# YixunLiang/UniTEX

Hardware: AMD Instinct MI355X
Metric: denoising-steps/sec (higher is better)
Workload: dtype bf16

## Files before the change

### include/unitex_hip.h

```cpp
#ifndef UNITEX_HIP_H
#define UNITEX_HIP_H
#include <stdint.h>
#ifdef __cplusplus
extern "C" {
#endif
#if defined(__GNUC__)
#pragma GCC visibility push(default)
#endif

#define UTX_VERSION 100

typedef struct utx_ctx utx_ctx;
typedef void* utx_stream;

int utx_version(void);
int utx_init(int device, utx_ctx** ctx);
void utx_free(utx_ctx* ctx);
const char* utx_last_error(utx_ctx* ctx);

int utx_set_option(const char* name, int value);
int utx_get_option(const char* name, int* value);
int utx_is_ablation_build(void);


int utx_attn_fwd_bf16(utx_ctx* ctx, const void* q, const void* k, const void* vt, void* o,
                      long q_hs, long q_ss, long k_hs, long k_ss, long vt_hs, long vt_ds, long o_ss,
                      int H, int S, float softmax_scale, utx_stream stream);
int utx_attn_fwd_bf16_kb(utx_ctx* ctx, const void* q, const void* k, const void* vt, void* o,
                         long q_hs, long q_ss, long k_hs, long k_ss, long vt_hs, long vt_ds, long o_ss,
                         int H, int S, float softmax_scale, float key_bias_log2, int key_bias_period, utx_stream stream);
int utx_attn_fwd_bf16_kbq(utx_ctx* ctx, const void* q, const void* k, const void* vt, void* o,
                          long q_hs, long q_ss, long k_hs, long k_ss, long vt_hs, long vt_ds, long o_ss,
                          int H, int S_q, int S_kv, float softmax_scale, float key_bias_log2, int key_bias_period, utx_stream stream);
int utx_attn_fwd_bf16_ws(utx_ctx* ctx, const void* q, const void* k, const void* vt, void* o,
                         long q_hs, long q_ss, long k_hs, long k_ss, long vt_hs, long vt_ds, long o_ss,
                         int H, int S_q, int S_kv, float softmax_scale, float key_bias_log2, int key_bias_period,
                         void* work, size_t work_bytes, utx_stream stream);
size_t utx_attn_workspace_bytes(utx_ctx* ctx, int H, int S_q, int S_kv);

int utx_quant_vt_mx8(utx_ctx* ctx, const void* vt, void* v8, void* vs, int H, int S_pad, utx_stream stream);
int utx_attn_fwd_fp8(utx_ctx* ctx, const void* q8, const void* qs, const void* k8, const void* ks, const void* v8t, const void* vs, void* o, long o_ss,
                     int H, int S_q, int S_kv, int S_pad, float key_bias_log2, int key_bias_period, utx_stream stream);
int utx_attn_fwd_fp8_ws(utx_ctx* ctx, const void* q8, const void* qs, const void* k8, const void* ks, const void* v8t, const void* vs, void* o, long o_ss,
                        int H, int S_q, int S_kv, int S_pad, float key_bias_log2, int key_bias_period, void* work, size_t work_bytes, utx_stream stream);
int utx_attn_plan(int H, int S_q, int S_kv, int n_cus, int out[4]);
int utx_attn_fwd_bf16_blk(utx_ctx* ctx, const void* q, const void* k, const void* vt, void* o,
                          long q_hs, long q_ss, long k_hs, long k_ss, long vt_hs, long vt_ds, long o_ss,
                          int H, int S_q, int S_kv, float softmax_scale, float key_bias_log2, int key_bias_period,
                          void* work, size_t work_bytes, int blk_rows, long q_bs, long k_bs, long vt_bs, utx_stream stream);

typedef struct utx_gemm_desc {
    const void* A; long lda;
    const void* B; long ldb;
    const void* A2; long lda2;
    const void* B2; long ldb2;
    int M, N, K, K2;
    int lora_n_limit;
    int lora_seg_n;
    float alpha;
    const void* bias;
    int gelu_from;
    const void* gate;
    const void* res; long ldres;
    void* C; long ldc;
    int n_split; void* C1; long ldc1;
    int ntn;
    int conv_Hi, conv_Wi, conv_Wo, conv_cin_log2, conv_stride, conv_pad, conv_up;
    const void* zero_page;
    const void* a_scale; long lds_a;
    const void* b_scale; long lds_b;
    int mx8;
    int qk_cols;
    int qk_tok_off;
    float qk_eps, qk_q_scale;
    const void* qk_wq; const void* qk_wk;
    const float* qk_cos; const float* qk_sin;
    void* qk_Qh; void* qk_Kh; long qk_hs;
    void* sk_work; size_t sk_work_bytes;
    void* q_out; long ldq_out;
    void* qs_out; long qs_out_rb;
    int q_out_kt0;
} utx_gemm_desc;
int utx_gemm_bf16(utx_ctx* ctx, const utx_gemm_desc* d, utx_stream stream);
size_t utx_gemm_streamk_workspace_bytes(utx_ctx* ctx);
int utx_gemm_plan(const utx_gemm_desc* d, int n_cus, int out[4]);

int utx_quant_mx8(utx_ctx* ctx, const void* x, long ldx, void* q, long ldq, void* s, long lds, int M, int K, utx_stream stream);
int utx_quant_mx8_packed(utx_ctx* ctx, const void* x, long ldx, void* q, long ldq, void* s, long row_blocks, int M, int K, utx_stream stream);

typedef struct utx_gemv_desc {
    const void* x; long ldx;
    const void* W; long ldw;
    const void* bias;
    void* y; long ldy;
    int M, N, K;
    int silu_in, silu_out;
} utx_gemv_desc;
int utx_gemv_bf16(utx_ctx* ctx, const utx_gemv_desc* d, utx_stream stream);

size_t utx_group_norm_workspace_bytes(void);
int utx_group_norm(utx_ctx* ctx, const void* x, long npix, int C, const void* gamma, const void* beta, float eps, int silu,
                   void* y, void* work, utx_stream stream);
int utx_softmax_rows(utx_ctx* ctx, void* s, long nrow, long ld, int ncol, utx_stream stream);
int utx_conv3x3_thin(utx_ctx* ctx, const void* x, int H, int W, int Cin, const void* wt, const void* bias, int Cout, void* y,
                     utx_stream stream);

typedef struct utx_qkv_post_desc {
    const void* qkv; long ld;
    int q_col, k_col, v_col;
    const void* wq; const void* wk;
    const float* cosb; const float* sinb;
    void* Qh; void* Kh; void* Vt;
    long hs_qk, hs_v, S_pad;
    int n_tok, tok_off, H;
    float eps;
    float q_scale;
    int heads_per_group;
    long gs_qk, gs_v;
    int skip_qk;
    int sub_heads;
    long gs2_qk, gs2_v;
} utx_qkv_post_desc;
int utx_qkv_post(utx_ctx* ctx, const utx_qkv_post_desc* d, utx_stream stream);

int utx_sp_unpack_qkv(utx_ctx* ctx, const void* recv, int P, int Hp, int S_loc, void* q, void* k, void* vt, utx_stream stream);
int utx_sp_unpack_qkv_dedup(utx_ctx* ctx, const void* recv, int P, int Hp, int S_loc, int text_rows, void* q, void* k, void* vt, utx_stream stream);
int utx_sp_unpack_o(utx_ctx* ctx, const void* recv, int P, int Hp, int S_loc, void* out, long ld, utx_stream stream);
int utx_sp_unpack_o_cols(utx_ctx* ctx, const void* recv, int P, int Hp, int S_loc, void* out, long ld, long src_cols, utx_stream stream);

typedef struct utx_ln_mod_desc {
    const void* x; long ldx;
    const void* shift; const void* scale;
    void* y; long ldy;
    int n_tok, D;
    float eps;
    void* q; long ldq;
    void* qs; long qs_row_blocks;
} utx_ln_mod_desc;
int utx_ln_mod(utx_ctx* ctx, const utx_ln_mod_desc* d, utx_stream stream);

typedef struct utx_sched_desc {
    void* x; const void* v; const void* cond;
    long n_noise_elems, n_total_elems;
    float dsigma;
} utx_sched_desc;
int utx_sched_step(utx_ctx* ctx, const utx_sched_desc* d, utx_stream stream);



int utx_transform_points(utx_ctx* ctx, const float* verts, int V, const float* mvp, int n_views,
                         float* clip, float* ndc, utx_stream stream);

long utx_rasterize_workspace_bytes(int F, int H, int W);
int utx_rasterize(utx_ctx* ctx, const float* pos, const int* tri, int F, int H, int W, float* rast,
                  void* work, utx_stream stream);

int utx_interpolate(utx_ctx* ctx, const float* attr, int C, const float* rast, const int* tri, long npix,
                    float* out, utx_stream stream);

int utx_condition_shade(utx_ctx* ctx, const float* rast, const float* nrm, const float* pos, const float* bg3_host,
                        long npix, void* out_normal, void* out_ccm, void* out_alpha, utx_stream stream);

int utx_face_normals(utx_ctx* ctx, const float* verts, const int* faces, int F, float* out, utx_stream stream);

int utx_texture_shade(utx_ctx* ctx, const float* rast, const float* uv, const int* tri, const float* tex, int Ht, int Wt,
                      const float* bg3_host, long npix, void* out, utx_stream stream);

// ... 153 lines not shown
                          int H, int W, void* tmp, void* vis_out, utx_stream stream);

int utx_composite(utx_ctx* ctx, const float* colors, const void* vis, const int* order_host, int n_order, long T,
                  float* atlas, void* winner, utx_stream stream);

int utx_seam_mask(utx_ctx* ctx, const void* winner, const float* rast2d, int H, int W, void* tmp, void* seam, utx_stream stream);
int utx_seam_mask_sized(utx_ctx* ctx, const void* winner, const float* rast2d, int H, int W, int k_boundary, int k_boundary_blur, void* tmp, void* seam,
                        utx_stream stream);

long utx_nn_fill_workspace_bytes(long T);
int utx_nn_fill(utx_ctx* ctx, const float* pos, const void* winner, const float* rast2d, long T, float* atlas,
                int* nn_index, void* work, long work_bytes, utx_stream stream);

int utx_view_visibility(utx_ctx* ctx, const float* attr6, const float* rast, const float* fnormal, const float* dirs, int n, int H, int W,
                        float grad_thr, float cos_thr, int radius, void* tmp, void* vis, float* alpha, utx_stream stream);
int utx_view_visibility_persp(utx_ctx* ctx, const float* attr6, const float* rast, const float* fnormal, const float* eyes, int n, int H, int W,
                              float grad_thr, float cos_thr, int radius, void* tmp, void* vis, float* alpha, utx_stream stream);

typedef struct utx_knn_desc {
    const float* src_pos; const float* src_attr; const float* src_nrm; const unsigned char* src_mask; long N;
    const float* dst_pos; const float* dst_nrm; const unsigned char* dst_mask; long M;
    int k, C, mode;
    float* out_attr; int* out_idx; float* out_d2;
} utx_knn_desc;
long utx_knn_workspace_bytes(long N);
int utx_knn(utx_ctx* ctx, const utx_knn_desc* d, void* work, long work_bytes, utx_stream stream);


long utx_fps_workspace_bytes(long N);
int utx_fps(utx_ctx* ctx, const float* pos, const void* mask, long N, int M, int start, int* out_idx, float* out_d2, void* work, long work_bytes,
            utx_stream stream);
int utx_sample_edges_equal_steps(utx_ctx* ctx, const float* verts, const int* edges, const int* edge_ids, const float* start, const float* length, int E,
                                 float total, long N, float* samples, int* edge_index, float* edge_t, utx_stream stream);
int utx_sample_surface(utx_ctx* ctx, const float* verts, const int* faces, const float* cum, int F, long N, unsigned long long seed, float* samples,
                       int* face_index, float* uvw, utx_stream stream);

int utx_lens_blur_seam(utx_ctx* ctx, const float* src, const void* seam, int H, int W, const float* k49_host, float* dst, utx_stream stream);
int utx_gaussian_blur_seam(utx_ctx* ctx, const float* src, const void* seam, int H, int W, int ksize, const float* w1_host, float* dst, utx_stream stream);

long utx_pull_push_workspace_bytes(int H, int W);
int utx_pull_push(utx_ctx* ctx, const float* kd, const void* mask, int H, int W, float* out, void* work, utx_stream stream);


int utx_backproject_vis(utx_ctx* ctx, const utx_backproject_desc* d, const float* eyes, int sample_mode, utx_bvh* bvh, utx_stream stream);
int utx_composite_winner(utx_ctx* ctx, const void* vis, int n_views, const int* order_host, int n_order, long T, void* winner, utx_stream stream);
int utx_gather_winner(utx_ctx* ctx, const float* rast2d, const int* faces, const float* vndc, const float* images, const void* winner, long T, int V,
                      int n_views, int H, int W, int C, int sample_mode, float* atlas, utx_stream stream);
int utx_nn_fill_c(utx_ctx* ctx, const float* pos, const void* winner, const float* rast2d, long T, int C, float* atlas, int* nn_index,
                  void* work, long work_bytes, utx_stream stream);
int utx_lens_blur_seam_c(utx_ctx* ctx, const float* src, const void* seam, int H, int W, int C, const float* k49_host, float* dst, utx_stream stream);
int utx_gaussian_blur_seam_c(utx_ctx* ctx, const float* src, const void* seam, int H, int W, int C, int ksize, const float* w1_host, float* dst, utx_stream stream);
long utx_pull_push_workspace_bytes_c(int H, int W, int C);
int utx_pull_push_c(utx_ctx* ctx, const float* kd, const void* mask, int H, int W, int C, float* out, void* work, utx_stream stream);

int utx_to_u8(utx_ctx* ctx, const float* src, long n_rows, long row_elems, int flip, void* dst, utx_stream stream);


int utx_chart_flood(utx_ctx* ctx, const int* adj, const int* bucket, int F, int* chart, int* flag, utx_stream stream);

typedef struct utx_plan utx_plan;
int utx_plan_create(utx_ctx* ctx, utx_plan** out);
void utx_plan_free(utx_plan* plan);
int utx_plan_size(const utx_plan* plan);
int utx_plan_add_gemm(utx_plan* plan, const utx_gemm_desc* d);
int utx_plan_add_gemv(utx_plan* plan, const utx_gemv_desc* d);
int utx_plan_add_ln_mod(utx_plan* plan, const utx_ln_mod_desc* d);
int utx_plan_add_qkv_post(utx_plan* plan, const utx_qkv_post_desc* d);
int utx_plan_add_attn(utx_plan* plan, const void* q, const void* k, const void* vt, void* o, long q_hs, long q_ss, long k_hs, long k_ss, long vt_hs,
                      long vt_ds, long o_ss, int H, int S_q, int S_kv, float softmax_scale, float key_bias_log2, int key_bias_period, void* work,
                      size_t work_bytes);
int utx_plan_add_quant_mx8(utx_plan* plan, const void* x, long ldx, void* q, long ldq, void* s, long lds_or_row_blocks, int M, int K, int packed);
int utx_plan_add_add3(utx_plan* plan, const void* a, const void* b, const void* c, void* out, int n);
int utx_plan_add_quant_vt_mx8(utx_plan* plan, const void* vt, void* v8, void* vs, int H, int S_pad);
int utx_plan_add_attn_fp8(utx_plan* plan, const void* q8, const void* qs, const void* k8, const void* ks, const void* v8t, const void* vs, void* o, long o_ss,
                          int H, int S_q, int S_kv, int S_pad, float key_bias_log2, int key_bias_period);
int utx_plan_add_attn_fp8_ws(utx_plan* plan, const void* q8, const void* qs, const void* k8, const void* ks, const void* v8t, const void* vs, void* o, long o_ss,
                             int H, int S_q, int S_kv, int S_pad, float key_bias_log2, int key_bias_period, void* work, size_t work_bytes);
int utx_plan_fork(utx_plan* plan);
int utx_plan_main(utx_plan* plan);
int utx_plan_join(utx_plan* plan);
int utx_plan_run(utx_plan* plan, utx_stream stream, int* failed_entry);
int utx_plan_run_range(utx_plan* plan, int begin, int end, utx_stream stream, int* failed_entry);
int utx_plan_assign_sk(utx_plan* plan, void* sk_work, size_t sk_work_bytes, int n_cus);
int utx_plan_entry(const utx_plan* plan, int i, int* kind, int* side, void* buf, size_t cap);

typedef struct utx_dit_linear {
    const void* w; const void* b;
    const void* lora_A; const void* lora_B;
    float lora_alpha; int lora_rp; int lora_nseg;
    const void* q; const void* s; long lds_s; const void* sp; int sp_row_blocks;
} utx_dit_linear;
typedef struct utx_dit_double_block {
    utx_dit_linear qkv_x, qkv_c, out_x, out_c, ff1_x, ff2_x, ff1_c, ff2_c;
    const void* nq; const void* nk; const void* naq; const void* nak;
    int mod_x, mod_c;
} utx_dit_double_block;
typedef struct utx_dit_single_block {
    utx_dit_linear qkvm, out;
    const void* nq; const void* nk;
    int mod;
} utx_dit_single_block;
typedef struct utx_dit_weights {
    utx_dit_linear x_embedder, context_embedder, proj_out, t_lin1, t_lin2, g_lin1, g_lin2, p_lin1, p_lin2, mod;
    const utx_dit_double_block* dbl; const utx_dit_single_block* sgl;
    int mod_out, n_mod;
} utx_dit_weights;
typedef struct utx_dit_config {
    int num_heads, num_double, num_single, in_channels, joint_dim, pooled_dim, mlp_ratio, guidance_embeds;
    int S_txt, S_img, n_out;
    float key_bias_log2; int key_bias_period;
    int two_streams, n_cus, lora_rank_padded;
    int fp8, fp8_fuse_quant;
} utx_dit_config;
typedef struct utx_dit_workspace {
    void *lat, *enc, *pooled, *tproj, *gproj, *e1, *e_t, *e_g, *e_p, *temb, *mod, *h, *xn, *qkv, *cat, *attn, *out;
    float *cos, *sin;
    void *Qh, *Kh, *Vt, *T, *Tc;
    void* sk_work; size_t sk_work_bytes;
    void* attn_work; size_t attn_work_bytes;
    void *aq, *as_rm, *asp; int asp_row_blocks;
    void *aq2, *asp2; int asp2_row_blocks;
} utx_dit_workspace;
int utx_dit_load(utx_ctx* ctx, const utx_dit_config* cfg, const utx_dit_weights* weights, const utx_dit_workspace* ws, utx_plan** out);
int utx_dit_step(utx_plan* plan, utx_stream stream, int* failed_entry);

int utx_mesh_decimate_qem(const float* verts, int V, const int* faces, int F, int target_faces, double boundary_weight,
                          float* verts_out, int* faces_out, int* V_out, int* F_out);

int utx_abi_sizes(int* out, int n);

#if defined(__GNUC__)
#pragma GCC visibility pop
#endif
#ifdef __cplusplus
}
#endif
#endif
```

### unitex_amd/_lib.py

```python
import ctypes as C
import os

_HERE = os.path.dirname(os.path.abspath(__file__))
LIB_PATH = os.path.join(_HERE, "lib", "libunitex_hip.so")

c_void_p, c_long, c_int, c_float = C.c_void_p, C.c_long, C.c_int, C.c_float


class GemmDesc(C.Structure):
    _fields_ = [("A", c_void_p), ("lda", c_long), ("B", c_void_p), ("ldb", c_long),
                ("A2", c_void_p), ("lda2", c_long), ("B2", c_void_p), ("ldb2", c_long),
                ("M", c_int), ("N", c_int), ("K", c_int), ("K2", c_int),
                ("lora_n_limit", c_int), ("lora_seg_n", c_int), ("alpha", c_float),
                ("bias", c_void_p), ("gelu_from", c_int), ("gate", c_void_p),
                ("res", c_void_p), ("ldres", c_long), ("C", c_void_p), ("ldc", c_long),
                ("n_split", c_int), ("C1", c_void_p), ("ldc1", c_long), ("ntn", c_int),
                ("conv_Hi", c_int), ("conv_Wi", c_int), ("conv_Wo", c_int), ("conv_cin_log2", c_int),
                ("conv_stride", c_int), ("conv_pad", c_int), ("conv_up", c_int), ("zero_page", c_void_p),
                ("a_scale", c_void_p), ("lds_a", c_long), ("b_scale", c_void_p), ("lds_b", c_long), ("mx8", c_int),
                ("qk_cols", c_int), ("qk_tok_off", c_int), ("qk_eps", c_float), ("qk_q_scale", c_float),
                ("qk_wq", c_void_p), ("qk_wk", c_void_p), ("qk_cos", c_void_p), ("qk_sin", c_void_p),
                ("qk_Qh", c_void_p), ("qk_Kh", c_void_p), ("qk_hs", c_long),
                ("sk_work", c_void_p), ("sk_work_bytes", C.c_size_t),
                ("q_out", c_void_p), ("ldq_out", c_long), ("qs_out", c_void_p), ("qs_out_rb", c_long), ("q_out_kt0", c_int)]


class GemvDesc(C.Structure):
    _fields_ = [("x", c_void_p), ("ldx", c_long), ("W", c_void_p), ("ldw", c_long),
                ("bias", c_void_p), ("y", c_void_p), ("ldy", c_long),
                ("M", c_int), ("N", c_int), ("K", c_int), ("silu_in", c_int), ("silu_out", c_int)]


class QkvPostDesc(C.Structure):
    _fields_ = [("qkv", c_void_p), ("ld", c_long), ("q_col", c_int), ("k_col", c_int), ("v_col", c_int),
                ("wq", c_void_p), ("wk", c_void_p), ("cosb", c_void_p), ("sinb", c_void_p),
                ("Qh", c_void_p), ("Kh", c_void_p), ("Vt", c_void_p),
                ("hs_qk", c_long), ("hs_v", c_long), ("S_pad", c_long),
                ("n_tok", c_int), ("tok_off", c_int), ("H", c_int), ("eps", c_float), ("q_scale", c_float),
                ("heads_per_group", c_int), ("gs_qk", c_long), ("gs_v", c_long), ("skip_qk", c_int),
                ("sub_heads", c_int), ("gs2_qk", c_long), ("gs2_v", c_long)]


class LnModDesc(C.Structure):
    _fields_ = [("x", c_void_p), ("ldx", c_long), ("shift", c_void_p), ("scale", c_void_p),
                ("y", c_void_p), ("ldy", c_long), ("n_tok", c_int), ("D", c_int), ("eps", c_float),
                ("q", c_void_p), ("ldq", c_long), ("qs", c_void_p), ("qs_row_blocks", c_long)]


class SchedDesc(C.Structure):
    _fields_ = [("x", c_void_p), ("v", c_void_p), ("cond", c_void_p),
                ("n_noise_elems", c_long), ("n_total_elems", c_long), ("dsigma", c_float)]


class BackprojectDesc(C.Structure):
    _fields_ = [("rast2d", c_void_p), ("verts", c_void_p), ("faces", c_void_p), ("fnormal", c_void_p),
                ("vndc", c_void_p), ("dirs", c_void_p), ("images", c_void_p),
                ("color", c_void_p), ("rayvis", c_void_p), ("alphaok", c_void_p),
                ("T_h", c_int), ("T_w", c_int), ("V", c_int), ("n_views", c_int), ("H", c_int), ("W", c_int),
                ("view_begin", c_int), ("view_count", c_int), ("cos_thresh", c_float), ("two_sqrt3", c_float)]


class KnnDesc(C.Structure):
    _fields_ = [("src_pos", c_void_p), ("src_attr", c_void_p), ("src_nrm", c_void_p), ("src_mask", c_void_p), ("N", c_long),
                ("dst_pos", c_void_p), ("dst_nrm", c_void_p), ("dst_mask", c_void_p), ("M", c_long),
                ("k", c_int), ("C", c_int), ("mode", c_int),
                ("out_attr", c_void_p), ("out_idx", c_void_p), ("out_d2", c_void_p)]


class DitLinear(C.Structure):
    _fields_ = [("w", c_void_p), ("b", c_void_p), ("lora_A", c_void_p), ("lora_B", c_void_p), ("lora_alpha", c_float), ("lora_rp", c_int), ("lora_nseg", c_int),
                ("q", c_void_p), ("s", c_void_p), ("lds_s", c_long), ("sp", c_void_p), ("sp_row_blocks", c_int)]


class DitDoubleBlock(C.Structure):
    _fields_ = [(n, DitLinear) for n in ("qkv_x", "qkv_c", "out_x", "out_c", "ff1_x", "ff2_x", "ff1_c", "ff2_c")] + \
               [("nq", c_void_p), ("nk", c_void_p), ("naq", c_void_p), ("nak", c_void_p), ("mod_x", c_int), ("mod_c", c_int)]


class DitSingleBlock(C.Structure):
    _fields_ = [("qkvm", DitLinear), ("out", DitLinear), ("nq", c_void_p), ("nk", c_void_p), ("mod", c_int)]


class DitWeights(C.Structure):
    _fields_ = [(n, DitLinear) for n in ("x_embedder", "context_embedder", "proj_out", "t_lin1", "t_lin2", "g_lin1", "g_lin2", "p_lin1", "p_lin2", "mod")] + \
               [("dbl", C.POINTER(DitDoubleBlock)), ("sgl", C.POINTER(DitSingleBlock)), ("mod_out", c_int), ("n_mod", c_int)]


class DitConfig(C.Structure):
    _fields_ = [(n, c_int) for n in ("num_heads", "num_double", "num_single", "in_channels", "joint_dim", "pooled_dim", "mlp_ratio", "guidance_embeds",
                                     "S_txt", "S_img", "n_out")] + [("key_bias_log2", c_float), ("key_bias_period", c_int), ("two_streams", c_int), ("n_cus", c_int),
                                                                     ("lora_rank_padded", c_int), ("fp8", c_int), ("fp8_fuse_quant", c_int)]


class DitWorkspace(C.Structure):
    _fields_ = [(n, c_void_p) for n in ("lat", "enc", "pooled", "tproj", "gproj", "e1", "e_t", "e_g", "e_p", "temb", "mod", "h", "xn", "qkv", "cat", "attn", "out",
                                        "cos", "sin", "Qh", "Kh", "Vt", "T", "Tc")] + \
               [("sk_work", c_void_p), ("sk_work_bytes", C.c_size_t), ("attn_work", c_void_p), ("attn_work_bytes", C.c_size_t),
                ("aq", c_void_p), ("as_rm", c_void_p), ("asp", c_void_p), ("asp_row_blocks", c_int), ("aq2", c_void_p), ("asp2", c_void_p), ("asp2_row_blocks", c_int)]


ABI_STRUCTS = [GemmDesc, GemvDesc, QkvPostDesc, LnModDesc, SchedDesc, BackprojectDesc, KnnDesc, DitLinear, DitDoubleBlock, DitSingleBlock, DitWeights, DitConfig,
               DitWorkspace]

SYMBOLS = {
    "utx_version": (c_int, []),
    "utx_init": (c_int, [c_int, C.POINTER(c_void_p)]),
    "utx_free": (None, [c_void_p]),
    "utx_last_error": (C.c_char_p, [c_void_p]),
    "utx_abi_sizes": (c_int, [C.POINTER(c_int), c_int]),
    "utx_plan_create": (c_int, [c_void_p, C.POINTER(c_void_p)]),
    "utx_plan_free": (None, [c_void_p]),
    "utx_plan_size": (c_int, [c_void_p]),
    "utx_plan_add_gemm": (c_int, [c_void_p, C.POINTER(GemmDesc)]),
    "utx_plan_add_gemv": (c_int, [c_void_p, C.POINTER(GemvDesc)]),
    "utx_plan_add_ln_mod": (c_int, [c_void_p, C.POINTER(LnModDesc)]),
    "utx_plan_add_qkv_post": (c_int, [c_void_p, C.POINTER(QkvPostDesc)]),
    "utx_plan_add_attn": (c_int, [c_void_p] * 5 + [c_long] * 7 + [c_int, c_int, c_int, c_float, c_float, c_int, c_void_p, C.c_size_t]),
    "utx_plan_add_quant_mx8": (c_int, [c_void_p, c_void_p, c_long, c_void_p, c_long, c_void_p, c_long, c_int, c_int, c_int]),
    "utx_plan_add_add3": (c_int, [c_void_p, c_void_p, c_void_p, c_void_p, c_void_p, c_int]),
    "utx_plan_add_quant_vt_mx8": (c_int, [c_void_p, c_void_p, c_void_p, c_void_p, c_int, c_int]),
    "utx_plan_add_attn_fp8": (c_int, [c_void_p] * 8 + [c_long, c_int, c_int, c_int, c_int, c_float, c_int]),
    "utx_plan_add_attn_fp8_ws": (c_int, [c_void_p] * 8 + [c_long, c_int, c_int, c_int, c_int, c_float, c_int, c_void_p, C.c_size_t]),
    "utx_plan_fork": (c_int, [c_void_p]),
    "utx_plan_main": (c_int, [c_void_p]),
    "utx_plan_join": (c_int, [c_void_p]),
    "utx_plan_run": (c_int, [c_void_p, c_void_p, C.POINTER(c_int)]),
    "utx_plan_run_range": (c_int, [c_void_p, c_int, c_int, c_void_p, C.POINTER(c_int)]),
    "utx_plan_assign_sk": (c_int, [c_void_p, c_void_p, C.c_size_t, c_int]),
    "utx_plan_entry": (c_int, [c_void_p, c_int, C.POINTER(c_int), C.POINTER(c_int), c_void_p, C.c_size_t]),
    "utx_dit_load": (c_int, [c_void_p, C.POINTER(DitConfig), C.POINTER(DitWeights), C.POINTER(DitWorkspace), C.POINTER(c_void_p)]),
    "utx_dit_step": (c_int, [c_void_p, c_void_p, C.POINTER(c_int)]),
    "utx_mesh_decimate_qem": (c_int, [c_void_p, c_int, c_void_p, c_int, c_int, C.c_double, c_void_p, c_void_p, C.POINTER(c_int), C.POINTER(c_int)]),
    "utx_set_option": (c_int, [C.c_char_p, c_int]),
    "utx_get_option": (c_int, [C.c_char_p, C.POINTER(c_int)]),
    "utx_is_ablation_build": (c_int, []),
    "utx_attn_fwd_bf16": (c_int, [c_void_p] * 5 + [c_long] * 7 + [c_int, c_int, c_float, c_void_p]),
    "utx_attn_fwd_bf16_kb": (c_int, [c_void_p] * 5 + [c_long] * 7 + [c_int, c_int, c_float, c_float, c_int, c_void_p]),
    "utx_attn_fwd_bf16_kbq": (c_int, [c_void_p] * 5 + [c_long] * 7 + [c_int, c_int, c_int, c_float, c_float, c_int, c_void_p]),
    "utx_attn_fwd_bf16_ws": (c_int, [c_void_p] * 5 + [c_long] * 7 + [c_int, c_int, c_int, c_float, c_float, c_int, c_void_p, C.c_size_t, c_void_p]),
    "utx_attn_fwd_bf16_blk": (c_int, [c_void_p] * 5 + [c_long] * 7 + [c_int, c_int, c_int, c_float, c_float, c_int, c_void_p, C.c_size_t, c_int, c_long, c_long, c_long,
                                      c_void_p]),
    "utx_attn_workspace_bytes": (C.c_size_t, [c_void_p, c_int, c_int, c_int]),
    "utx_quant_vt_mx8": (c_int, [c_void_p, c_void_p, c_void_p, c_void_p, c_int, c_int, c_void_p]),
    "utx_attn_fwd_fp8": (c_int, [c_void_p] * 8 + [c_long, c_int, c_int, c_int, c_int, c_float, c_int, c_void_p]),
    "utx_attn_fwd_fp8_ws": (c_int, [c_void_p] * 8 + [c_long, c_int, c_int, c_int, c_int, c_float, c_int, c_void_p, C.c_size_t, c_void_p]),
    "utx_attn_plan": (c_int, [c_int, c_int, c_int, c_int, c_void_p]),
    "utx_gemm_bf16": (c_int, [c_void_p, C.POINTER(GemmDesc), c_void_p]),
    "utx_gemm_streamk_workspace_bytes": (C.c_size_t, [c_void_p]),
    "utx_gemm_plan": (c_int, [C.POINTER(GemmDesc), c_int, C.POINTER(c_int * 4)]),
    "utx_quant_mx8": (c_int, [c_void_p, c_void_p, c_long, c_void_p, c_long, c_void_p, c_long, c_int, c_int, c_void_p]),
    "utx_quant_mx8_packed": (c_int, [c_void_p, c_void_p, c_long, c_void_p, c_long, c_void_p, c_long, c_int, c_int, c_void_p]),
    "utx_gemv_bf16": (c_int, [c_void_p, C.POINTER(GemvDesc), c_void_p]),
    "utx_group_norm_workspace_bytes": (c_long, []),
    "utx_group_norm": (c_int, [c_void_p, c_void_p, c_long, c_int, c_void_p, c_void_p, c_float, c_int, c_void_p, c_void_p, c_void_p]),
    "utx_softmax_rows": (c_int, [c_void_p, c_void_p, c_long, c_long, c_int, c_void_p]),
    "utx_conv3x3_thin": (c_int, [c_void_p, c_void_p, c_int, c_int, c_int, c_void_p, c_void_p, c_int, c_void_p, c_void_p]),
    "utx_qkv_post": (c_int, [c_void_p, C.POINTER(QkvPostDesc), c_void_p]),
    "utx_sp_unpack_qkv": (c_int, [c_void_p, c_void_p, c_int, c_int, c_int, c_void_p, c_void_p, c_void_p, c_void_p]),
    "utx_sp_unpack_qkv_dedup": (c_int, [c_void_p, c_void_p, c_int, c_int, c_int, c_int, c_void_p, c_void_p, c_void_p, c_void_p]),
    "utx_sp_unpack_o": (c_int, [c_void_p, c_void_p, c_int, c_int, c_int, c_void_p, c_long, c_void_p]),
    "utx_sp_unpack_o_cols": (c_int, [c_void_p, c_void_p, c_int, c_int, c_int, c_void_p, c_long, c_long, c_void_p]),
    "utx_ln_mod": (c_int, [c_void_p, C.POINTER(LnModDesc), c_void_p]),
    "utx_sched_step": (c_int, [c_void_p, C.POINTER(SchedDesc), c_void_p]),
    "utx_transform_points": (c_int, [c_void_p, c_void_p, c_int, c_void_p, c_int, c_void_p, c_void_p, c_void_p]),
    "utx_rasterize_workspace_bytes": (c_long, [c_int, c_int, c_int]),
    "utx_rasterize": (c_int, [c_void_p, c_void_p, c_void_p, c_int, c_int, c_int, c_void_p, c_void_p, c_void_p]),
    "utx_interpolate": (c_int, [c_void_p, c_void_p, c_int, c_void_p, c_void_p, c_long, c_void_p, c_void_p]),
    "utx_condition_shade": (c_int, [c_void_p, c_void_p, c_void_p, c_void_p, C.POINTER(c_float), c_long, c_void_p, c_void_p, c_void_p, c_void_p]),
    "utx_face_normals": (c_int, [c_void_p, c_void_p, c_void_p, c_int, c_void_p, c_void_p]),
    "utx_texture_shade": (c_int, [c_void_p, c_void_p, c_void_p, c_void_p, c_void_p, c_int, c_int, C.POINTER(c_float), c_long, c_void_p, c_void_p]),
    "utx_gbuffer_shade": (c_int, [c_void_p, c_int, c_void_p, c_void_p, c_void_p, c_int, c_void_p, c_int, C.POINTER(c_float), c_long, c_void_p, c_void_p, c_void_p]),
    "utx_gbuffer_range": (c_int, [c_void_p, c_int, c_void_p, c_void_p, c_void_p, c_int, c_long, c_void_p, c_void_p, c_void_p]),
    "utx_camera_normals": (c_int, [c_void_p, c_void_p, c_int, c_void_p, c_int, c_void_p, c_void_p]),
    "utx_uv_gbuffer": (c_int, [c_void_p, c_void_p, c_void_p, c_void_p, c_void_p, c_void_p, c_void_p, c_int, c_int, c_int, c_int, C.c_uint, C.POINTER(c_void_p), c_void_p]),
    "utx_screen_gbuffer": (c_int, [c_void_p] * 7 + [c_int] + [c_void_p] * 3 + [c_int] * 5 + [C.POINTER(c_void_p), C.POINTER(c_int), c_int, c_int, c_float, c_void_p, c_void_p,
                                   C.c_uint, C.POINTER(c_void_p), c_void_p]),
    "utx_cubemap_table": (c_int, [c_int, c_float, c_void_p, c_void_p]),
    "utx_latlong_to_cubemap": (c_int, [c_void_p, c_void_p, c_int, c_int, c_int, c_void_p, c_void_p]),
    "utx_cubemap_diffuse": (c_int, [c_void_p, c_void_p, c_int, c_void_p, c_void_p, c_void_p]),
    "utx_cubemap_specular": (c_int, [c_void_p, c_void_p, c_int, c_void_p, c_void_p, c_float, c_float, c_void_p, c_void_p]),
    "utx_dfg_lut": (c_int, [c_void_p, c_int, c_int, c_void_p, c_void_p]),
    "utx_cube_sample": (c_int, [c_void_p, c_void_p, c_int, c_void_p, c_long, c_void_p, c_void_p]),
    "utx_pbr_forward": (c_int, [c_void_p, c_void_p, c_int, c_void_p, c_void_p, c_void_p, c_int, c_void_p, c_void_p, c_int, c_void_p, c_int, c_void_p, c_int, c_long,
                                c_void_p, c_void_p, c_void_p]),
    "utx_pbr_shade": (c_int, [c_void_p, c_void_p, c_void_p, c_void_p, c_void_p, c_void_p, c_void_p, c_int, c_int, c_void_p, c_int, c_int, C.POINTER(c_float),
                              c_void_p, c_int, c_void_p, c_int, c_void_p, c_int, c_float, c_float, C.POINTER(c_float), c_long, c_void_p, c_void_p, c_void_p]),
    "utx_pbr_shading_normal": (c_int, [c_void_p, c_void_p, c_int, c_void_p, c_void_p, c_void_p, c_void_p, c_void_p, c_long, c_void_p, c_void_p]),
    "utx_pbr_shade_nm": (c_int, [c_void_p, c_void_p, c_void_p, c_void_p, c_void_p, c_void_p, c_void_p, c_void_p, c_void_p, c_int, c_int, c_void_p, c_int, c_int,
                                 c_void_p, c_int, c_int, C.POINTER(c_float), c_void_p, c_int, c_void_p, c_int, c_void_p, c_int, c_float, c_float, C.POINTER(c_float),
                                 c_long, c_void_p, c_void_p, c_void_p]),
    "utx_bvh_build": (c_int, [c_void_p, c_void_p, c_int, c_void_p, c_int, C.POINTER(c_void_p), c_void_p]),
    "utx_bvh_workspace_bytes": (C.c_size_t, [c_int]),
    "utx_bvh_build_ws": (c_int, [c_void_p, c_void_p, c_int, c_void_p, c_int, c_void_p, C.c_size_t, C.POINTER(c_void_p), c_void_p]),
    "utx_bvh_free": (None, [c_void_p]),
    "utx_bvh_arrays": (c_int, [c_void_p, C.POINTER(c_void_p), C.POINTER(c_void_p), C.POINTER(c_void_p), C.POINTER(c_void_p)]),
    "utx_bvh_trace": (c_int, [c_void_p, c_void_p, c_void_p, c_void_p, c_long, c_void_p, c_void_p]),
    "utx_visible_faces_rays": (c_int, [c_void_p] * 4 + [c_int, c_void_p, c_int, c_int, c_int, c_void_p, c_void_p, c_void_p]),
    "utx_visible_faces_raster": (c_int, [c_void_p, c_void_p, c_int, c_int, c_int, c_int, c_void_p, c_void_p]),
    "utx_erode_faces": (c_int, [c_void_p, c_void_p, c_void_p, c_int, c_int, c_int, c_int, c_void_p, c_void_p]),
    "utx_visible_vertices": (c_int, [c_void_p, c_void_p, c_void_p, c_int, c_int, c_int, c_void_p, c_void_p]),
    "utx_uv_project": (c_int, [c_void_p, c_void_p, c_void_p, c_int, c_void_p, c_void_p] + [c_int] * 4 + [c_void_p] + [c_int] * 4 + [c_void_p, c_int, c_int, c_float] +
                       [c_void_p] * 5),
    "utx_view_weight_maps": (c_int, [c_void_p, c_void_p, c_void_p, c_int, c_int, c_int, c_int, c_void_p, c_void_p, c_void_p, c_void_p]),
    "utx_vertex_project": (c_int, [c_void_p, c_void_p, c_int, c_void_p, c_int, c_void_p, c_void_p, c_void_p, c_int, c_int, c_void_p, c_int, c_int, c_void_p, c_void_p,
                                   c_int, c_void_p, c_void_p, c_void_p]),
    "utx_vertex_project_blend": (c_int, [c_void_p, c_void_p, c_int, c_void_p, c_int, c_void_p, c_void_p, c_void_p, c_int, c_int, c_void_p, c_int, c_int, c_void_p,
                                         c_void_p, c_int, c_void_p, c_void_p, c_float, c_int, c_float, c_float, c_void_p, c_void_p, c_void_p]),
    "utx_vertex_inpaint_step": (c_int, [c_void_p, c_void_p, c_void_p, c_void_p, c_int, c_void_p, c_void_p, c_void_p, c_void_p, c_void_p, c_void_p]),
    "utx_uv_bake": (c_int, [c_void_p, c_void_p, c_void_p, c_int, c_void_p, c_void_p, c_int, c_int, c_int, c_int, c_void_p, c_void_p, c_void_p, c_int, c_void_p,
                            c_void_p, c_int, c_void_p, c_void_p, c_int, c_float, c_int, c_float, c_float, c_void_p, c_void_p, c_void_p]),
    "utx_uv_dilation_step": (c_int, [c_void_p, c_void_p, c_void_p, c_int, c_int, c_int, c_int, c_void_p, c_void_p, c_void_p, c_void_p]),
    "utx_bvh_trace_count": (c_int, [c_void_p, c_void_p, c_void_p, c_void_p, c_long, c_void_p, c_void_p, c_void_p]),
    "utx_bvh_depth": (c_int, [c_void_p]),
    "utx_backproject": (c_int, [c_void_p, C.POINTER(BackprojectDesc), c_void_p, c_void_p]),
    "utx_backproject_persp": (c_int, [c_void_p, C.POINTER(BackprojectDesc), c_void_p, c_void_p, c_void_p]),
    "utx_backproject_sampled": (c_int, [c_void_p, C.POINTER(BackprojectDesc), c_void_p, c_int, c_void_p, c_void_p]),
    "utx_dilate_visibility": (c_int, [c_void_p, c_void_p, c_void_p, c_void_p, c_int, c_int, c_int, c_void_p, c_void_p, c_void_p]),
    "utx_composite": (c_int, [c_void_p, c_void_p, c_void_p, C.POINTER(c_int), c_int, c_long, c_void_p, c_void_p, c_void_p]),
    "utx_seam_mask": (c_int, [c_void_p, c_void_p, c_void_p, c_int, c_int, c_void_p, c_void_p, c_void_p]),
    "utx_seam_mask_sized": (c_int, [c_void_p, c_void_p, c_void_p, c_int, c_int, c_int, c_int, c_void_p, c_void_p, c_void_p]),
    "utx_view_visibility": (c_int, [c_void_p, c_void_p, c_void_p, c_void_p, c_void_p, c_int, c_int, c_int, c_float, c_float, c_int,
                                    c_void_p, c_void_p, c_void_p, c_void_p]),
    "utx_view_visibility_persp": (c_int, [c_void_p, c_void_p, c_void_p, c_void_p, c_void_p, c_int, c_int, c_int, c_float, c_float, c_int,
                                          c_void_p, c_void_p, c_void_p, c_void_p]),
    "utx_knn_workspace_bytes": (c_long, [c_long]),
    "utx_knn": (c_int, [c_void_p, C.POINTER(KnnDesc), c_void_p, c_long, c_void_p]),
    "utx_fps_workspace_bytes": (c_long, [c_long]),
    "utx_fps": (c_int, [c_void_p, c_void_p, c_void_p, c_long, c_int, c_int, c_void_p, c_void_p, c_void_p, c_long, c_void_p]),
    "utx_sample_edges_equal_steps": (c_int, [c_void_p, c_void_p, c_void_p, c_void_p, c_void_p, c_void_p, c_int, c_float, c_long, c_void_p, c_void_p, c_void_p, c_void_p]),
    "utx_sample_surface": (c_int, [c_void_p, c_void_p, c_void_p, c_void_p, c_int, c_long, C.c_ulonglong, c_void_p, c_void_p, c_void_p, c_void_p]),
    "utx_nn_fill_workspace_bytes": (c_long, [c_long]),
# ... 113 lines not shown
```

### unitex_amd/csrc/build.py

```python
import os
import subprocess
import sys
from concurrent.futures import ThreadPoolExecutor

HERE = os.path.dirname(os.path.abspath(__file__))
LIBDIR = os.path.normpath(os.path.join(HERE, "..", "lib"))
OBJDIR = os.path.join(HERE, "_obj")
HIPCC = os.environ.get("HIPCC", "/opt/rocm/bin/hipcc")
ARCH = "gfx950"

NO_PK = ["-Xclang", "-target-feature", "-Xclang", "-packed-fp32-ops"]

SOURCES = [
    ("attention.hip", []),
    ("attention_glds.hip", ["-fno-slp-vectorize"]),
    ("attention_q64.hip", []),
    ("attention_fp8.hip", NO_PK),
    ("gemm.hip", []),
    ("gemm_w4.hip", []),
    ("dit_elementwise.hip", ["-ffp-contract=off"] + NO_PK),
    ("vae.hip", NO_PK),
    ("capi.cpp", []),
    ("meshproc.cpp", []),
    ("plan.cpp", []),
    ("dit_plan.cpp", []),
]
GEOM = [
    ("raster.hip", ["-ffp-contract=off"]),
    ("gbuffer.hip", ["-ffp-contract=off"] + NO_PK),
    ("pbr.hip", ["-ffp-contract=off"] + NO_PK),
    ("bvh.hip", ["-ffp-contract=off"] + NO_PK),
    ("backproject.hip", ["-ffp-contract=off"] + NO_PK),
    ("vertex_bake.hip", ["-ffp-contract=off"] + NO_PK),
    ("uv_bake.hip", ["-ffp-contract=off"] + NO_PK),
    ("texture_post.hip", ["-ffp-contract=off"] + NO_PK),
    ("knn.hip", ["-ffp-contract=off"]),
    ("sampling.hip", ["-ffp-contract=off"]),
    ("unwrap.hip", []),
]
for s in GEOM:
    if os.path.exists(os.path.join(HERE, s[0])):
        SOURCES.append(s)

COMMON = ["--offload-arch=" + ARCH, "-O3", "-std=c++17", "-fPIC", "-fvisibility=hidden", "-I" + HERE,
          "-I" + os.path.normpath(os.path.join(HERE, "..", "..", "include")), "-x", "hip"]


def _newer(src, obj):
    if not os.path.exists(obj):
        return True
    t = os.path.getmtime(obj)
    deps = [src] + [os.path.join(HERE, h) for h in os.listdir(HERE) if h.endswith(".h") or h.endswith(".inc")]
    deps.append(os.path.normpath(os.path.join(HERE, "..", "..", "include", "unitex_hip.h")))
    return any(os.path.getmtime(d) > t for d in deps)


def _compile(item, objdir=None, defines=()):
    name, extra = item
    objdir = objdir or OBJDIR
    src = os.path.join(HERE, name)
    obj = os.path.join(objdir, name + ".o")
    if _newer(src, obj):
        cmd = [HIPCC] + COMMON + list(defines) + extra + ["-c", src, "-o", obj]
        r = subprocess.run(cmd, capture_output=True, text=True)
        if r.returncode != 0:
            raise RuntimeError("hipcc failed for %s:\n%s" % (name, r.stderr[-4000:]))
    return obj


def build(verbose=True, ablate=False):
    if ablate:
        gen = os.path.normpath(os.path.join(HERE, "..", "..", "tools", "gen_attn_q64.py"))
        r = subprocess.run([sys.executable, gen, "--variants", "--keep-default"], capture_output=True, text=True)
        if r.returncode != 0:
            raise RuntimeError("gen_attn_q64.py failed:\n" + r.stderr[-2000:])
    objdir = OBJDIR + ("_ablate" if ablate else "")
    defines = ["-DUTX_ABLATION"] if ablate else []
    os.makedirs(objdir, exist_ok=True)
    os.makedirs(LIBDIR, exist_ok=True)
    with ThreadPoolExecutor(max_workers=min(8, len(SOURCES))) as ex:
        objs = list(ex.map(lambda it: _compile(it, objdir, defines), SOURCES))
    out = os.path.join(LIBDIR, "libunitex_hip_ablate.so" if ablate else "libunitex_hip.so")
    if (not os.path.exists(out)) or any(os.path.getmtime(o) > os.path.getmtime(out) for o in objs):
        cmd = [HIPCC, "--offload-arch=" + ARCH, "-shared", "-fPIC", "-o", out] + objs
        r = subprocess.run(cmd, capture_output=True, text=True)
        if r.returncode != 0:
            raise RuntimeError("link failed:\n%s" % r.stderr[-4000:])
    if verbose:
        print("built", out)
    return out


if __name__ == "__main__":
    build(ablate="--ablate" in sys.argv)
    sys.exit(0)
```

### unitex_amd/csrc/capi.cpp

```cpp
#include <cstdint>
#include <hip/hip_runtime.h>
#include <stdio.h>
#include <string.h>
#include <string>
#include <stdlib.h>
#include <mutex>
#include <map>
#include <vector>
#include <utility>
#include "kernels.h"
#include "common.h"

UtxOptions g_utx_opt;

struct OptName { const char* name; int UtxOptions::*field; bool ablation; };
static const OptName kOptions[] = {
    {"UTX_ATTN_Q64", &UtxOptions::attn_q64, false},         {"UTX_ATTN_TAILSPLIT", &UtxOptions::attn_tailsplit, false},
    {"UTX_GEMM_GROUP_M", &UtxOptions::gemm_group_m, false}, {"UTX_GEMM_TILE", &UtxOptions::gemm_tile, false},
    {"UTX_GEMM_PERS_GRID", &UtxOptions::gemm_pers_grid, false}, {"UTX_GEMM_STREAMK", &UtxOptions::gemm_streamk, false},
    {"UTX_BVH_STACK_WALK", &UtxOptions::bvh_stack_walk, false}, {"UTX_BVH_PACKET", &UtxOptions::bvh_packet, false},
    {"UTX_ATTN_PEEL", &UtxOptions::attn_peel, false},             {"UTX_ATTN8_PEEL", &UtxOptions::attn8_peel, false},
    {"UTX_NN_GRID", &UtxOptions::nn_grid, false},                 {"UTX_GEMM_FASTK", &UtxOptions::gemm_fastk, false},
    {"UTX_ATTN_VAR", &UtxOptions::attn_var_abl, true},      {"UTX_ATTN_DEBUG", &UtxOptions::attn_debug_abl, true},
    {"UTX_GEMM_DEBUG", &UtxOptions::gemm_debug_abl, true},
// ... 138 lines not shown
                         long q_hs, long q_ss, long k_hs, long k_ss, long vt_hs, long vt_ds, long o_ss,
                         int H, int S, float softmax_scale, float key_bias_log2, int key_bias_period, utx_stream stream) {
    if (!q || !k || !vt || !o) return fail(ctx, -2, "utx_attn_fwd_bf16_kb");
    size_t wsb = 0; void* const ws = ctx_attn_ws(ctx, H, S, S, (hipStream_t)stream, &wsb);
    UTX_CALL(ctx, "utx_attn_fwd_bf16_kb",
             utx_launch_attn_fwd(q, k, vt, o, q_hs, q_ss, k_hs, k_ss, vt_hs, vt_ds, o_ss, H, S, S,
                                 softmax_scale, key_bias_log2, key_bias_period, ws, wsb, (hipStream_t)stream));
}

int utx_attn_fwd_bf16_kbq(utx_ctx* ctx, const void* q, const void* k, const void* vt, void* o,
                          long q_hs, long q_ss, long k_hs, long k_ss, long vt_hs, long vt_ds, long o_ss,
                          int H, int S_q, int S_kv, float softmax_scale, float key_bias_log2, int key_bias_period, utx_stream stream) {
    if (!q || !k || !vt || !o) return fail(ctx, -2, "utx_attn_fwd_bf16_kbq");
    size_t wsb = 0; void* const ws = (S_q > 0) ? ctx_attn_ws(ctx, H, S_q, S_kv, (hipStream_t)stream, &wsb) : nullptr;
    UTX_CALL(ctx, "utx_attn_fwd_bf16_kbq",
             utx_launch_attn_fwd(q, k, vt, o, q_hs, q_ss, k_hs, k_ss, vt_hs, vt_ds, o_ss, H, S_kv, S_q,
                                 softmax_scale, key_bias_log2, key_bias_period, ws, wsb, (hipStream_t)stream));
}

int utx_attn_fwd_bf16_ws(utx_ctx* ctx, const void* q, const void* k, const void* vt, void* o,
                         long q_hs, long q_ss, long k_hs, long k_ss, long vt_hs, long vt_ds, long o_ss,
                         int H, int S_q, int S_kv, float softmax_scale, float key_bias_log2, int key_bias_period,
                         void* work, size_t work_bytes, utx_stream stream) {
    if (!q || !k || !vt || !o) return fail(ctx, -2, "utx_attn_fwd_bf16_ws");
    UTX_CALL(ctx, "utx_attn_fwd_bf16_ws",
             utx_launch_attn_fwd(q, k, vt, o, q_hs, q_ss, k_hs, k_ss, vt_hs, vt_ds, o_ss, H, S_kv, S_q,
                                 softmax_scale, key_bias_log2, key_bias_period, work, work_bytes, (hipStream_t)stream));
}

int utx_attn_fwd_bf16_blk(utx_ctx* ctx, const void* q, const void* k, const void* vt, void* o,
                          long q_hs, long q_ss, long k_hs, long k_ss, long vt_hs, long vt_ds, long o_ss,
                          int H, int S_q, int S_kv, float softmax_scale, float key_bias_log2, int key_bias_period,
                          void* work, size_t work_bytes, int blk_rows, long q_bs, long k_bs, long vt_bs, utx_stream stream) {
    if (!q || !k || !vt || !o || blk_rows <= 0) return fail(ctx, -2, "utx_attn_fwd_bf16_blk");
    UTX_CALL(ctx, "utx_attn_fwd_bf16_blk",
             utx_launch_attn_fwd_blk(q, k, vt, o, q_hs, q_ss, k_hs, k_ss, vt_hs, vt_ds, o_ss, H, S_kv, S_q,
                                     softmax_scale, key_bias_log2, key_bias_period, work, work_bytes, blk_rows, q_bs, k_bs, vt_bs, (hipStream_t)stream));
}

int utx_quant_vt_mx8(utx_ctx* ctx, const void* vt, void* v8, void* vs, int H, int S_pad, utx_stream stream) {
    if (!vt || !v8 || !vs) return fail(ctx, -2, "utx_quant_vt_mx8");
    UTX_CALL(ctx, "utx_quant_vt_mx8", utx_launch_quant_vt_mx8(vt, v8, vs, H, S_pad, (hipStream_t)stream));
}

int utx_attn_fwd_fp8(utx_ctx* ctx, const void* q8, const void* qs, const void* k8, const void* ks, const void* v8t, const void* vs, void* o, long o_ss,
                     int H, int S_q, int S_kv, int S_pad, float key_bias_log2, int key_bias_period, utx_stream stream) {
    if (!q8 || !qs || !k8 || !ks || !v8t || !vs || !o) return fail(ctx, -2, "utx_attn_fwd_fp8");
    Attn8Params p;
    p.q8 = (const uint8_t*)q8; p.k8 = (const uint8_t*)k8; p.v8t = (const uint8_t*)v8t;
    p.qs = (const uint32_t*)qs; p.ks = (const uint32_t*)ks; p.vs = (const uint32_t*)vs;
    p.o = (bf16_t*)o; p.o_ss = o_ss; p.H = H; p.S = S_kv; p.Sq = S_q; p.S_pad = S_pad; p.nqb = 0;
    p.key_bias_log2 = key_bias_log2; p.key_bias_period = key_bias_period;
    p.work = (S_q > 0 && S_q <= S_kv) ? ctx_attn_ws(ctx, H, S_q, S_kv, (hipStream_t)stream, &p.work_bytes) : nullptr;
    if (!p.work) p.work_bytes = 0;
    UTX_CALL(ctx, "utx_attn_fwd_fp8", utx_launch_attn_fwd_fp8(&p, (hipStream_t)stream));
}

int utx_attn_fwd_fp8_ws(utx_ctx* ctx, const void* q8, const void* qs, const void* k8, const void* ks, const void* v8t, const void* vs, void* o, long o_ss,
                        int H, int S_q, int S_kv, int S_pad, float key_bias_log2, int key_bias_period, void* work, size_t work_bytes, utx_stream stream) {
    if (!q8 || !qs || !k8 || !ks || !v8t || !vs || !o) return fail(ctx, -2, "utx_attn_fwd_fp8_ws");
    Attn8Params p;
    p.q8 = (const uint8_t*)q8; p.k8 = (const uint8_t*)k8; p.v8t = (const uint8_t*)v8t;
    p.qs = (const uint32_t*)qs; p.ks = (const uint32_t*)ks; p.vs = (const uint32_t*)vs;
    p.o = (bf16_t*)o; p.o_ss = o_ss; p.H = H; p.S = S_kv; p.Sq = S_q; p.S_pad = S_pad; p.nqb = 0;
    p.key_bias_log2 = key_bias_log2; p.key_bias_period = key_bias_period;
    p.work = work; p.work_bytes = work ? work_bytes : 0;
    UTX_CALL(ctx, "utx_attn_fwd_fp8_ws", utx_launch_attn_fwd_fp8(&p, (hipStream_t)stream));
}

size_t utx_attn_workspace_bytes(utx_ctx* ctx, int H, int S_q, int S_kv) {
    (void)ctx;
    if (H <= 0 || S_kv <= 0 || S_q <= 0) return 0;
    return utx_attn_workspace_bytes_impl(H, S_q == S_kv ? 0 : S_q, S_kv, utx_ncu());
}

int utx_attn_plan(int H, int S_q, int S_kv, int n_cus, int out[4]) {
    if (!out || H <= 0 || S_kv <= 0 || S_q <= 0 || n_cus <= 0) return -2;
    options_from_env_once();
    utx_attn_split_plan_impl(H, S_q == S_kv ? 0 : S_q, S_kv, n_cus, out);
    return 0;
}

size_t utx_gemm_streamk_workspace_bytes(utx_ctx*) { return utx_gemm_streamk_workspace_bytes_impl(); }
int utx_gemm_plan(const utx_gemm_desc* d, int n_cus, int out[4]) {
    if (!d || !out || n_cus <= 0 || d->M <= 0 || d->N <= 0 || d->K <= 0) return -2;
    options_from_env_once();
    return utx_gemm_plan_impl(d, n_cus, d->sk_work != nullptr, out);
}
int utx_gemm_bf16(utx_ctx* ctx, const utx_gemm_desc* d, utx_stream stream) {
    if (!d || !d->A || !d->B || !d->C) return fail(ctx, -2, "utx_gemm_bf16");
    UTX_CALL(ctx, "utx_gemm_bf16", utx_launch_gemm_bf16(d, (hipStream_t)stream));
}

int utx_quant_mx8(utx_ctx* ctx, const void* x, long ldx, void* q, long ldq, void* sc, long lds, int M, int K, utx_stream stream) {
    if (!x || !q || !sc) return fail(ctx, -2, "utx_quant_mx8");
    UTX_CALL(ctx, "utx_quant_mx8", utx_launch_quant_mx8(x, ldx, q, ldq, sc, lds, M, K, (hipStream_t)stream));
}

int utx_quant_mx8_packed(utx_ctx* ctx, const void* x, long ldx, void* q, long ldq, void* sc, long row_blocks, int M, int K, utx_stream stream) {
    if (!x || !q || !sc) return fail(ctx, -2, "utx_quant_mx8_packed");
    UTX_CALL(ctx, "utx_quant_mx8_packed", utx_launch_quant_mx8_packed(x, ldx, q, ldq, sc, row_blocks, M, K, (hipStream_t)stream));
}

int utx_gemv_bf16(utx_ctx* ctx, const utx_gemv_desc* d, utx_stream stream) {
    if (!d || !d->x || !d->W || !d->y) return fail(ctx, -2, "utx_gemv_bf16");
    UTX_CALL(ctx, "utx_gemv_bf16", utx_launch_gemv_bf16(d, (hipStream_t)stream));
}

size_t utx_group_norm_workspace_bytes(void) { return utx_group_norm_workspace_bytes_impl(); }

int utx_group_norm(utx_ctx* ctx, const void* x, long npix, int C, const void* gamma, const void* beta, float eps, int silu,
                   void* y, void* work, utx_stream stream) {
    if (!x || !gamma || !beta || !y || !work) return fail(ctx, -2, "utx_group_norm");
    UTX_CALL(ctx, "utx_group_norm", utx_launch_group_norm(x, npix, C, gamma, beta, eps, silu, y, work, (hipStream_t)stream));
}

int utx_softmax_rows(utx_ctx* ctx, void* s, long nrow, long ld, int ncol, utx_stream stream) {
    if (!s) return fail(ctx, -2, "utx_softmax_rows");
    UTX_CALL(ctx, "utx_softmax_rows", utx_launch_softmax_rows(s, nrow, ld, ncol, (hipStream_t)stream));
}

int utx_conv3x3_thin(utx_ctx* ctx, const void* x, int H, int W, int Cin, const void* wt, const void* bias, int Cout, void* y,
                     utx_stream stream) {
    if (!x || !wt || !bias || !y) return fail(ctx, -2, "utx_conv3x3_thin");
    UTX_CALL(ctx, "utx_conv3x3_thin", utx_launch_conv3x3_thin(x, H, W, Cin, wt, bias, Cout, y, (hipStream_t)stream));
}

int utx_qkv_post(utx_ctx* ctx, const utx_qkv_post_desc* d, utx_stream stream) {
    if (!d || !d->qkv || !d->Qh || !d->Kh || !d->Vt || !d->cosb || !d->sinb || !d->wq || !d->wk)
        return fail(ctx, -2, "utx_qkv_post");
    UTX_CALL(ctx, "utx_qkv_post", utx_launch_qkv_post(d, (hipStream_t)stream));
}

int utx_sp_unpack_qkv(utx_ctx* ctx, const void* recv, int P, int Hp, int S_loc, void* q, void* k, void* vt, utx_stream stream) {
    if (!recv || !q || !k || !vt) return fail(ctx, -2, "utx_sp_unpack_qkv");
    UTX_CALL(ctx, "utx_sp_unpack_qkv", utx_launch_sp_unpack_qkv(recv, P, Hp, S_loc, 0, q, k, vt, (hipStream_t)stream));
}

int utx_sp_unpack_qkv_dedup(utx_ctx* ctx, const void* recv, int P, int Hp, int S_loc, int text_rows, void* q, void* k, void* vt, utx_stream stream) {
    if (!recv || !q || !k || !vt) return fail(ctx, -2, "utx_sp_unpack_qkv_dedup");
    UTX_CALL(ctx, "utx_sp_unpack_qkv_dedup", utx_launch_sp_unpack_qkv(recv, P, Hp, S_loc, text_rows, q, k, vt, (hipStream_t)stream));
}

int utx_sp_unpack_o(utx_ctx* ctx, const void* recv, int P, int Hp, int S_loc, void* out, long ld, utx_stream stream) {
    if (!recv || !out) return fail(ctx, -2, "utx_sp_unpack_o");
    UTX_CALL(ctx, "utx_sp_unpack_o", utx_launch_sp_unpack_o(recv, P, Hp, S_loc, out, ld, 0, (hipStream_t)stream));
}

int utx_sp_unpack_o_cols(utx_ctx* ctx, const void* recv, int P, int Hp, int S_loc, void* out, long ld, long src_cols, utx_stream stream) {
    if (!recv || !out || src_cols <= 0) return fail(ctx, -2, "utx_sp_unpack_o_cols");
    UTX_CALL(ctx, "utx_sp_unpack_o_cols", utx_launch_sp_unpack_o(recv, P, Hp, S_loc, out, ld, src_cols, (hipStream_t)stream));
}

int utx_ln_mod(utx_ctx* ctx, const utx_ln_mod_desc* d, utx_stream stream) {
    if (!d || !d->x || (!d->y && !d->q) || !d->shift || !d->scale) return fail(ctx, -2, "utx_ln_mod");
    UTX_CALL(ctx, "utx_ln_mod", utx_launch_ln_mod(d, (hipStream_t)stream));
}

int utx_sched_step(utx_ctx* ctx, const utx_sched_desc* d, utx_stream stream) {
    if (!d || !d->x || !d->v) return fail(ctx, -2, "utx_sched_step");
    UTX_CALL(ctx, "utx_sched_step", utx_launch_sched_step(d, (hipStream_t)stream));
}


int utx_transform_points(utx_ctx* ctx, const float* verts, int V, const float* mvp, int n_views, float* clip, float* ndc, utx_stream stream) {
    if (!verts || !mvp || !clip) return fail(ctx, -2, "utx_transform_points");
// ... 424 lines not shown
```

### unitex_amd/csrc/common.h

```cpp
#pragma once
#include <hip/hip_runtime.h>
#include <stdint.h>

typedef __attribute__((ext_vector_type(8))) __bf16 bf16x8;
typedef __attribute__((ext_vector_type(4))) __bf16 bf16x4;
typedef __attribute__((ext_vector_type(16))) float f32x16;
typedef __attribute__((ext_vector_type(4))) float f32x4;
typedef __attribute__((ext_vector_type(2))) float f32x2;
#ifndef UTX_BF16_T
#define UTX_BF16_T
typedef uint16_t bf16_t;
#endif

#define UTX_WAVE 64

__device__ __forceinline__ uint16_t f2bf(float f) {
    const __bf16 b = (__bf16)f;
    return __builtin_bit_cast(uint16_t, b);
}
__device__ __forceinline__ float bf2f(uint16_t h) { return __uint_as_float(((uint32_t)h) << 16); }
__device__ __forceinline__ uint32_t pack2bf(float lo, float hi) {
    typedef __attribute__((ext_vector_type(2))) __bf16 bf16x2_t;
    bf16x2_t v;
    v[0] = (__bf16)lo; v[1] = (__bf16)hi;
    return __builtin_bit_cast(uint32_t, v);
}
__device__ __forceinline__ float rbf(float f) { return bf2f(f2bf(f)); }

__device__ __forceinline__ float wave_sum(float v) {
#pragma unroll
    for (int o = 32; o > 0; o >>= 1) v += __shfl_xor(v, o, 64);
    return v;
}
__device__ __forceinline__ float wave_max(float v) {
#pragma unroll
    for (int o = 32; o > 0; o >>= 1) v = fmaxf(v, __shfl_xor(v, o, 64));
    return v;
}

__device__ __forceinline__ int xcd_remap(int bid, int nwg) {
    const int nx = 8;
    int xcd = bid % nx, j = bid / nx;
    int q = nwg / nx, r = nwg % nx;
    int base = (xcd < r) ? xcd * (q + 1) : r * (q + 1) + (xcd - r) * q;
    return base + j;
}

#include <atomic>
static inline int utx_device() { int d = 0; return (hipGetDevice(&d) == hipSuccess && d >= 0 && d < 64) ? d : -1; }
static inline int utx_ncu() {
    static std::atomic<int> tab[64] = {};
    const int d = utx_device();
    int n = d >= 0 ? tab[d].load(std::memory_order_relaxed) : 0;
    if (!n) {
        int cur = 0; hipDeviceProp_t pr;
        n = (hipGetDevice(&cur) == hipSuccess && hipGetDeviceProperties(&pr, cur) == hipSuccess) ? pr.multiProcessorCount : 256;
        if (d >= 0) tab[d].store(n, std::memory_order_relaxed);
    }
    return n;
}
#define UTX_ONCE_PER_DEVICE(flag_) static std::atomic<unsigned long long> flag_{0}; const int flag_##_dev = utx_device(); \
    if (flag_##_dev < 0 || !((flag_.load(std::memory_order_acquire) >> flag_##_dev) & 1ull))
#define UTX_ONCE_DONE(flag_) do { if (flag_##_dev >= 0) flag_.fetch_or(1ull << flag_##_dev, std::memory_order_release); } while (0)
```

### unitex_amd/csrc/dit_plan.cpp

```cpp
#include <hip/hip_runtime.h>
#include <math.h>
#include <string.h>
#include <vector>
#include "kernels.h"

extern "C" {
int utx_plan_assign_sk(utx_plan* p, void* sk_work, size_t sk_work_bytes, int n_cus);
}

namespace {
typedef const char* cptr;
inline cptr off(const void* base, long elems) { return (cptr)base + elems * 2; }

struct Builder {
    utx_plan* plan;
    const utx_dit_config& c;
    const utx_dit_workspace& w;
    int D, H, S, S_pad;
    long Kmax;
    int rc;
    Builder(utx_plan* p, const utx_dit_config& c_, const utx_dit_workspace& w_) : plan(p), c(c_), w(w_), rc(0) {
        H = c.num_heads; D = H * 128; S = c.S_txt + c.S_img; S_pad = (S + 63) / 64 * 64; Kmax = (long)(1 + c.mlp_ratio) * D;
    }
    void chk(int r) { if (r != 0 && rc == 0) rc = r; }

    utx_gemm_desc gemm_desc(const void* A, long lda, int M, int K, const void* B, int N, void* C, long ldc, const void* bias) const {
        utx_gemm_desc d; memset(&d, 0, sizeof(d));
        d.A = A; d.lda = lda; d.B = B; d.ldb = K;
        d.K2 = 0; d.lora_n_limit = 0; d.lora_seg_n = 128;
        d.M = M; d.N = N; d.K = K;
        d.alpha = 1.0f; d.bias = bias; d.gelu_from = N;
        d.C = C; d.ldc = ldc; d.n_split = N;
        return d;
    }
    void add_gemm(utx_gemm_desc d, bool main_stream) { (void)main_stream; chk(utx_plan_add_gemm(plan, &d)); }
    void linear(const utx_dit_linear& L, const void* A, long lda, int M, int K, int N, void* C, long ldc, bool main_stream, const void* T, int lora_limit, int lora_seg,
                int gelu_from = -1, const void* gate = nullptr, const void* res = nullptr, long ldres = 0, int n_split = -1, void* C1 = nullptr, long ldc1 = 0) {
        utx_gemm_desc d = gemm_desc(A, lda, M, K, L.w, N, C, ldc, L.b);
        if (L.lora_A && L.lora_rp > 0) {
            const int nr = L.lora_nseg * L.lora_rp;
            utx_gemm_desc d0 = gemm_desc(A, lda, M, K, L.lora_A, nr, (void*)T, 3L * c.lora_rank_padded, nullptr);
            d0.alpha = L.lora_alpha;
            add_gemm(d0, main_stream);
            d.A2 = T; d.lda2 = 3L * c.lora_rank_padded; d.B2 = L.lora_B; d.ldb2 = L.lora_rp; d.K2 = L.lora_rp;
            d.lora_n_limit = lora_limit > 0 ? lora_limit : N;
            d.lora_seg_n = lora_seg > 0 ? lora_seg : N;
        }
        if (gelu_from >= 0) d.gelu_from = gelu_from;
        d.gate = gate;
        if (gate) { d.res = res; d.ldres = ldres; }
        if (n_split >= 0) d.n_split = n_split;
        if (C1) { d.C1 = C1; d.ldc1 = ldc1; }
        add_gemm(d, main_stream);
    }
    void lnmod(const void* x, void* y, const void* shift, const void* scale, int n_tok, int mxq_row0 = -1) {
        utx_ln_mod_desc d; memset(&d, 0, sizeof(d));
        d.x = x; d.ldx = D; d.shift = shift; d.scale = scale; d.y = y; d.ldy = D; d.n_tok = n_tok; d.D = D; d.eps = 1e-6f;
        if (mxq_row0 >= 0) { d.q = (char*)w.aq + (long)mxq_row0 * Kmax; d.ldq = Kmax; d.qs = w.asp; d.qs_row_blocks = w.asp_row_blocks; }
        chk(utx_plan_add_ln_mod(plan, &d));
    }
    static bool shape_packed(int M, int N, int n_split = -1, int gelu_from = -1) {
        if (N % 256 || (n_split >= 0 && n_split < N && n_split % 256) || (gelu_from >= 0 && gelu_from < N && gelu_from % 256)) return false;
        return (long)((M + 255) / 256) * (N / 256) >= 192;
    }
    bool is_mx(const utx_dit_linear& L) const { return c.fp8 && L.q; }
    bool is_packed(const utx_dit_linear& L, int M, int N, int n_split = -1, int gelu_from = -1) const { return is_mx(L) && L.sp && shape_packed(M, N, n_split, gelu_from); }
    void quant(const void* x, long ldx, void* q, long ldq, void* s, long lds_or_rb, int M, int K, int packed) { chk(utx_plan_add_quant_mx8(plan, x, ldx, q, ldq, s, lds_or_rb, M, K, packed)); }
    struct MxOpt { int quant_cols; int a_col0; bool q_out; MxOpt() : quant_cols(-1), a_col0(0), q_out(false) {} };
    void linear_mx(const utx_dit_linear& L, bool packed, MxOpt o, int row0, const void* A, long lda, int M, int K, int N, void* C, long ldc, int gelu_from = -1,
                   const void* gate = nullptr, const void* res = nullptr, long ldres = 0, int n_split = -1, void* C1 = nullptr, long ldc1 = 0) {
        char* aqv = (char*)w.aq + (long)row0 * Kmax + (packed ? o.a_col0 : 0);
        utx_gemm_desc d = gemm_desc(aqv, Kmax, M, K, L.q, N, C, ldc, L.b);
        if (packed) {
            char* asv = (char*)w.asp + (long)(o.a_col0 / 128) * w.asp_row_blocks * 512;
            const int nq = o.quant_cols < 0 ? K : o.quant_cols;
            if (nq > 0) quant(A, lda, aqv, Kmax, asv, w.asp_row_blocks, M, nq, 1);
            d.a_scale = asv; d.lds_a = w.asp_row_blocks; d.b_scale = L.sp; d.lds_b = L.sp_row_blocks; d.mx8 = 2;
            if (o.q_out) { d.q_out = (char*)w.aq + (long)row0 * Kmax + D; d.ldq_out = Kmax; d.qs_out = w.asp; d.qs_out_rb = w.asp_row_blocks; d.q_out_kt0 = D / 128; }
        } else {
            char* asv = (char*)w.as_rm + (long)row0 * (Kmax / 32);
            quant(A, lda, aqv, Kmax, asv, Kmax / 32, M, K, 0);
            d.a_scale = asv; d.lds_a = Kmax / 32; d.b_scale = L.s; d.lds_b = L.lds_s; d.mx8 = 1;
        }
        if (gelu_from >= 0) d.gelu_from = gelu_from;
        d.gate = gate;
        if (gate) { d.res = res; d.ldres = ldres; }
        if (n_split >= 0) d.n_split = n_split;
        if (C1) { d.C1 = C1; d.ldc1 = ldc1; }
        add_gemm(d, true);
    }
// ... 105 lines not shown
        const bool f_sgl = fuse && p_qkvm && p_out;
        b.lnmod(h, (void*)xn, chunk(o, 0), chunk(o, 1), S, f_sgl ? 0 : -1);
        if (pruned && c.fp8 && B.qkvm.q && B.qkvm.sp && B.out.q && B.out.sp && Builder::shape_packed(n_out, D) && Builder::shape_packed(S, 2 * D)) {
            if (!ws->aq2 || !ws->asp2 || ws->asp2_row_blocks < (n_out + 127) / 128) { b.chk(-2); break; }
            const int r0 = S_txt, r1 = S_txt + n_out;
            const utx_dit_linear& L = B.qkvm;
            cptr Wq = (cptr)L.q, bm = (cptr)L.b;
            const long Kmax = b.Kmax;
            auto sp_rows = [&](const utx_dit_linear& X, int row) { return (const void*)((cptr)X.sp + (long)(row / 128) * 512); };
            auto mx_desc = [&](const void* A, int M, int K, const void* Bq, int N, void* Cc, long ldc, const void* bias, const void* as_, int a_rb, const void* bs_, int b_rb) {
                utx_gemm_desc d = b.gemm_desc(A, Kmax, M, K, Bq, N, Cc, ldc, bias);
                d.a_scale = as_; d.lds_a = a_rb; d.b_scale = bs_; d.lds_b = b_rb; d.mx8 = 2;
                return d;
            };
            b.quant(xn, D, ws->aq, Kmax, ws->asp, ws->asp_row_blocks, S, D, 1);
            b.add_gemm(mx_desc(ws->aq, S, D, Wq + (long)D * D, 2 * D, (void*)off(qkv, D), 3L * D, off(bm, D), ws->asp, ws->asp_row_blocks, sp_rows(L, D), L.sp_row_blocks), true);
            b.quant(off(xn, (long)r0 * D), D, ws->aq2, Kmax, ws->asp2, ws->asp2_row_blocks, n_out, D, 1);
            b.add_gemm(mx_desc(ws->aq2, n_out, D, Wq, D, (void*)off(qkv, (long)r0 * 3 * D), 3L * D, bm, ws->asp2, ws->asp2_row_blocks, sp_rows(L, 0), L.sp_row_blocks), true);
            {
                utx_gemm_desc d = mx_desc(ws->aq2, n_out, D, Wq + 3L * D * D, MR * D, (void*)off(cat, (long)r0 * ldcat + D), ldcat, off(bm, 3L * D), ws->asp2, ws->asp2_row_blocks,
                                          sp_rows(L, 3 * D), L.sp_row_blocks);
                d.gelu_from = 0;
                b.add_gemm(d, true);
            }
            b.qkvpost(qkv, B.nq, B.nk, S, 0);
            b.attn((void*)off(cat, (long)r0 * ldcat), ldcat, r0, r1);
            b.quant(off(cat, (long)r0 * ldcat), ldcat, ws->aq2, Kmax, ws->asp2, ws->asp2_row_blocks, n_out, (int)Kmax, 1);
            {
                utx_gemm_desc d = mx_desc(ws->aq2, n_out, (int)Kmax, B.out.q, D, (void*)off(h, (long)r0 * D), D, B.out.b, ws->asp2, ws->asp2_row_blocks, B.out.sp, B.out.sp_row_blocks);
                d.gate = chunk(o, 2); d.res = off(h, (long)r0 * D); d.ldres = D;
                b.add_gemm(d, true);
            }
            continue;
        }
        if (pruned) {
            const int r0 = S_txt, r1 = S_txt + n_out;
            const utx_dit_linear& L = B.qkvm;
            cptr Wm = (cptr)L.w, bm = (cptr)L.b;
            const bool lora = L.lora_A && L.lora_rp > 0;
            const int R = L.lora_rp;
            const long ldT = 3L * c.lora_rank_padded;
            if (lora) {
                utx_gemm_desc d0 = b.gemm_desc(xn, D, S, D, L.lora_A, 3 * R, (void*)T, ldT, nullptr);
                d0.alpha = L.lora_alpha;
                b.add_gemm(d0, true);
            }
            {
                utx_gemm_desc d = b.gemm_desc(xn, D, S, D, off(Wm, (long)D * D), 2 * D, (void*)off(qkv, D), 3L * D, off(bm, D));
                if (lora) { d.A2 = off(T, R); d.lda2 = ldT; d.B2 = off(L.lora_B, (long)D * R); d.ldb2 = R; d.K2 = R; d.lora_n_limit = 2 * D; d.lora_seg_n = D; }
                b.add_gemm(d, true);
            }
            {
                utx_gemm_desc d = b.gemm_desc(off(xn, (long)r0 * D), D, r1 - r0, D, Wm, D, (void*)off(qkv, (long)r0 * 3 * D), 3L * D, bm);
                if (lora) { d.A2 = off(T, (long)r0 * ldT); d.lda2 = ldT; d.B2 = L.lora_B; d.ldb2 = R; d.K2 = R; d.lora_n_limit = D; d.lora_seg_n = D; }
                b.add_gemm(d, true);
            }
            {
                utx_gemm_desc d = b.gemm_desc(off(xn, (long)r0 * D), D, r1 - r0, D, off(Wm, 3L * D * D), MR * D, (void*)off(cat, (long)r0 * ldcat + D), ldcat, off(bm, 3L * D));
                d.gelu_from = 0;
                b.add_gemm(d, true);
            }
            b.qkvpost(qkv, B.nq, B.nk, S, 0);
            b.attn((void*)off(cat, (long)r0 * ldcat), ldcat, r0, r1);
            {
                utx_gemm_desc d = b.gemm_desc(off(cat, (long)r0 * ldcat), ldcat, r1 - r0, (1 + MR) * D, B.out.w, D, (void*)off(h, (long)r0 * D), D, B.out.b);
                d.gate = chunk(o, 2); d.res = off(h, (long)r0 * D); d.ldres = D;
                b.add_gemm(d, true);
            }
            continue;
        }
        Builder::MxOpt o_qkvm, o_out;
        if (f_sgl) { o_qkvm.quant_cols = 0; o_qkvm.q_out = true; o_out.quant_cols = D; }
        if (x_qkvm) b.linear_mx(B.qkvm, p_qkvm, o_qkvm, 0, xn, D, S, D, (3 + MR) * D, (void*)qkv, 3L * D, 3 * D, nullptr, nullptr, 0, 3 * D, (void*)off(cat, D), ldcat);
        else b.linear(B.qkvm, xn, D, S, D, (3 + MR) * D, (void*)qkv, 3L * D, true, T, 3 * D, D, 3 * D, nullptr, nullptr, 0, 3 * D, (void*)off(cat, D), ldcat);
        b.qkvpost(qkv, B.nq, B.nk, S, 0);
        b.attn((void*)cat, ldcat, 0, S);
        if (x_out) b.linear_mx(B.out, p_out, o_out, 0, cat, ldcat, S, (1 + MR) * D, D, (void*)h, D, -1, chunk(o, 2), h, D);
        else b.linear(B.out, cat, ldcat, S, (1 + MR) * D, D, (void*)h, D, true, T, 0, 0, -1, chunk(o, 2), h, D);
    }
    b.lnmod(h_x, xn_x, chunk(wt->mod_out, 1), chunk(wt->mod_out, 0), n_out);
    b.linear(wt->proj_out, xn_x, D, n_out, D, c.in_channels, ws->out, c.in_channels, true, nullptr, 0, 0);
    if (b.rc) { utx_plan_free(plan); return b.rc; }
    utx_plan_assign_sk(plan, ws->sk_work, ws->sk_work_bytes, ncu);
    *out = plan;
    return 0;
}

extern "C" int utx_dit_step(utx_plan* plan, utx_stream stream, int* failed_entry) { return utx_plan_run(plan, stream, failed_entry); }
```

### unitex_amd/csrc/gemm.hip

```cpp
#include "common.h"
#include "kernels.h"
#include <stdlib.h>

#define GM_BK 64
#define GM_GROUP_M 4

__device__ __forceinline__ float gelu_tanh(float x) {
    const float k0 = 0.7978845608028654f, k1 = 0.044715f;
    const float u = k0 * (x + k1 * x * x * x);
    return x * __builtin_amdgcn_rcpf(1.0f + __expf(-2.0f * u));
}

__device__ __forceinline__ void glds16(const bf16_t* g, char* lds) {
    __builtin_amdgcn_global_load_lds((const __attribute__((address_space(1))) void*)g,
                                     (__attribute__((address_space(3))) void*)lds, 16, 0, 0);
}


#define GM_RES_LOAD1(it_, rowexpr_) rq##it_ = *reinterpret_cast<const uint4*>(pres + (long)(rowexpr_) * p.ldres + gn0);
#define GM_ROW_PASS1(it_, guard_)                                                                                \
    {                                                                                                            \
        const int ml = rrow0 + RPP * (it_);                                                                      \
        const int gm = m0 + 128 * chunk + ml;                                                                    \
        if (guard_) {                                                                                            \
            uint4 yv = *reinterpret_cast<const uint4*>(smem + ml * CROW + rslot * 16);                           \
            if (pgate) {                                                                                         \
                uint32_t yw[4] = {yv.x, yv.y, yv.z, yv.w};                                                       \
                const uint32_t rw[4] = {rq##it_.x, rq##it_.y, rq##it_.z, rq##it_.w};                             \
                _Pragma("unroll") for (int c = 0; c < 4; ++c) {                                                  \
                    const float y0 = bf2f((uint16_t)(yw[c] & 0xffff)), y1 = bf2f((uint16_t)(yw[c] >> 16));       \
                    const float r0 = bf2f((uint16_t)(rw[c] & 0xffff)), r1 = bf2f((uint16_t)(rw[c] >> 16));       \
                    const float o0 = r0 + rbf(gv[2 * c] * y0);                                                   \
                    const float o1 = r1 + rbf(gv[2 * c + 1] * y1);                                               \
                    yw[c] = pack2bf(o0, o1);                                                                     \
                }                                                                                                \
                yv = make_uint4(yw[0], yw[1], yw[2], yw[3]);                                                     \
            }                                                                                                    \
            *reinterpret_cast<uint4*>(cbase + (long)gm * ldc + cn) = yv;                                         \
        }                                                                                                        \
    }

typedef __attribute__((ext_vector_type(8))) int gm_i32x8;
template <int BM, int BN, int NWM, int NWN, bool CONV, bool MX8 = false>
__global__ __launch_bounds__(64 * NWM * NWN, 2) void gemm_bf16_kernel(GemmParams p) {
    constexpr int NW = NWM * NWN, NT = 64 * NW;
    constexpr int WMR = BM / NWM, WNR = BN / NWN;
    constexpr int MI = WMR / 32, NI = WNR / 32;
    constexpr int A_BYTES = BM * GM_BK * 2, B_BYTES = BN * GM_BK * 2, STAGE = A_BYTES + B_BYTES;
    constexpr int CROW = BN * 2 + 16;
    static_assert(BM / 8 / NW == 4 && BN / 8 / NW == 4, "4 A + 4 B global_load_lds per thread per K-step");
    extern __shared__ __attribute__((aligned(16))) char smem[];
    const bf16_t* pA = (const bf16_t*)p.A; const bf16_t* pB = (const bf16_t*)p.B;
    const bf16_t* pA2 = (const bf16_t*)p.A2; const bf16_t* pB2 = (const bf16_t*)p.B2;
    const bf16_t* pbias = (const bf16_t*)p.bias; const bf16_t* pgate = (const bf16_t*)p.gate;
    const bf16_t* pres = (const bf16_t*)p.res;
    bf16_t* pC = (bf16_t*)p.C; bf16_t* pC1 = (bf16_t*)p.C1;
    const int tid = threadIdx.x;
    const int lane = tid & 63;
    const int wave = __builtin_amdgcn_readfirstlane(tid >> 6);
    const int wm = wave / NWN, wn = wave % NWN;
    const int l31 = lane & 31, lh = lane >> 5;

    const int w = xcd_remap(blockIdx.x, gridDim.x);
    const int ntn = p.ntn & 0xffff, group_m = (p.ntn >> 16) & 0xff;
    const int ntm_ = (p.M + BM - 1) / BM;
    const int per_group = group_m * ntn;
    const int grp = w / per_group, rem = w - grp * per_group;
    const int first_tm = grp * group_m;
    const int gsize = (ntm_ - first_tm < group_m) ? ntm_ - first_tm : group_m;
    const int tm = first_tm + rem % gsize, tn = rem / gsize;
    const int m0 = tm * BM, n0 = tn * BN;

    const int nk1 = p.K / GM_BK;
    const bool lora = (p.K2 > 0) && (n0 < p.lora_n_limit);
    const int nk = nk1 + (lora ? p.K2 / GM_BK : 0);
    const long a2_off = lora ? (long)(n0 / p.lora_seg_n) * p.K2 : 0;

    const int srow_in = lane >> 3, sslot = lane & 7;
#define GM_SRC(j_)                                                                                       \
    const int srow##j_ = 8 * (wave + NW * (j_)) + srow_in;                                              \
    const int schunk##j_ = (sslot ^ ((srow##j_ >> 1) & 7)) * 8;                                          \
    const int sgm##j_ = (m0 + srow##j_ > p.M - 1) ? p.M - 1 : m0 + srow##j_;                             \
    const int sgn##j_ = (n0 + srow##j_ > p.N - 1) ? p.N - 1 : n0 + srow##j_;                             \
    const bf16_t* pa##j_ = pA + (long)sgm##j_ * p.lda + schunk##j_;                                      \
    const bf16_t* pb##j_ = pB + (long)sgn##j_ * p.ldb + schunk##j_;
    GM_SRC(0) GM_SRC(1) GM_SRC(2) GM_SRC(3)
    const bf16_t* pzero = (const bf16_t*)p.zero_page;
    const int chlim = CONV ? (p.conv_Hi << p.conv_up) : 0, cwlim = CONV ? (p.conv_Wi << p.conv_up) : 0;
#define GM_CONV_PIX(j_)                                                                                  \
    const int coy##j_ = CONV ? (sgm##j_ / p.conv_Wo) * p.conv_stride - p.conv_pad : 0;                   \
    const int cox##j_ = CONV ? (sgm##j_ % p.conv_Wo) * p.conv_stride - p.conv_pad : 0;
    GM_CONV_PIX(0) GM_CONV_PIX(1) GM_CONV_PIX(2) GM_CONV_PIX(3)
#define GM_CONV_PTR(j_)                                                                                  \
    {                                                                                                    \
// ... 153 lines not shown
                        const uint2 braw = bq[ni][a];
                        bv[0] = bf2f((uint16_t)(braw.x & 0xffff)); bv[1] = bf2f((uint16_t)(braw.x >> 16));
                        bv[2] = bf2f((uint16_t)(braw.y & 0xffff)); bv[3] = bf2f((uint16_t)(braw.y >> 16));
                    }
                    const bool do_gelu = (n0 + nl) >= p.gelu_from;
#pragma unroll
                    for (int mi = 0; mi < MI; ++mi) {
                        float y[4];
#pragma unroll
                        for (int c = 0; c < 4; ++c) {
                            float v = rbf(acc[ni][mi][4 * a + c] * p.alpha + bv[c]);
                            if (do_gelu) v = gelu_tanh(v);
                            y[c] = v;
                        }
                        uint2 o; o.x = pack2bf(y[0], y[1]); o.y = pack2bf(y[2], y[3]);
                        const int ml = wm * WMR + mi * 32 + l31 - 128 * chunk;
                        *reinterpret_cast<uint2*>(smem + ml * CROW + nl * 2) = o;
                    }
                }
            }
        }
        __syncthreads();
        if (gn0 < p.N) {
            GM_ROW_PASS1(0, gm < p.M) GM_ROW_PASS1(1, gm < p.M) GM_ROW_PASS1(2, gm < p.M) GM_ROW_PASS1(3, gm < p.M)
            GM_ROW_PASS1(4, gm < p.M) GM_ROW_PASS1(5, gm < p.M) GM_ROW_PASS1(6, gm < p.M) GM_ROW_PASS1(7, gm < p.M)
        }
    }
}


__device__ __forceinline__ float silu_f(float v) { return v / (1.0f + __expf(-v)); }

__global__ __launch_bounds__(256) void gemv_bf16_kernel(GemvParams p) {
    const int lane = threadIdx.x & 63;
    const int n = blockIdx.x * 4 + (threadIdx.x >> 6);
    if (n >= p.N) return;
    const bf16_t* wrow = (const bf16_t*)p.W + (long)n * p.ldw;
    const bf16_t* pbias = (const bf16_t*)p.bias;
    for (int m = 0; m < p.M; ++m) {
        const bf16_t* xr = (const bf16_t*)p.x + (long)m * p.ldx;
        float s = 0.f;
        for (int k = lane * 8; k < p.K; k += 64 * 8) {
            const uint4 wv = *reinterpret_cast<const uint4*>(wrow + k);
            const uint4 xv = *reinterpret_cast<const uint4*>(xr + k);
            const uint32_t ww[4] = {wv.x, wv.y, wv.z, wv.w};
            const uint32_t xw[4] = {xv.x, xv.y, xv.z, xv.w};
#pragma unroll
            for (int c = 0; c < 4; ++c) {
                float x0 = bf2f((uint16_t)(xw[c] & 0xffff)), x1 = bf2f((uint16_t)(xw[c] >> 16));
                if (p.silu_in) { x0 = rbf(silu_f(x0)); x1 = rbf(silu_f(x1)); }
                s += x0 * bf2f((uint16_t)(ww[c] & 0xffff));
                s += x1 * bf2f((uint16_t)(ww[c] >> 16));
            }
        }
        s = wave_sum(s);
        if (lane == 0) {
            float v = s + (pbias ? bf2f(pbias[n]) : 0.f);
            v = rbf(v);
            if (p.silu_out) v = silu_f(v);
            ((bf16_t*)p.y)[(long)m * p.ldy + n] = f2bf(v);
        }
    }
}

template <int BM, int BN, int NWM, int NWN, bool CONV = false, bool MX8 = false>
static int launch_gemm(GemmParams p, hipStream_t stream, int group_env) {
    constexpr int LDS = 2 * (BM + BN) * GM_BK * 2;
    UTX_ONCE_PER_DEVICE(attr_set) {
        if (hipFuncSetAttribute(reinterpret_cast<const void*>(gemm_bf16_kernel<BM, BN, NWM, NWN, CONV, MX8>),
                                hipFuncAttributeMaxDynamicSharedMemorySize, LDS) != hipSuccess) return -3;
        UTX_ONCE_DONE(attr_set);
    }
    const int ntm = (p.M + BM - 1) / BM;
    const int ntn = (p.N + BN - 1) / BN;
    int group_m = group_env > 0 ? group_env : GM_GROUP_M;
    if (group_m > ntm) group_m = ntm;
    p.ntn = ntn | (group_m << 16);
    hipLaunchKernelGGL((gemm_bf16_kernel<BM, BN, NWM, NWN, CONV, MX8>), dim3(ntm * ntn), dim3(64 * NWM * NWN), LDS, stream, p);
    return hipGetLastError() == hipSuccess ? 0 : -4;
}

static bool gemm_tile_known() {
    const int t = g_utx_opt.gemm_tile;
    return t == 0 || t == 128 || t == 2564;
}

extern "C" int utx_gemm_plan_impl(const GemmParams* pp, int ncu, int sk_has_work, int out[4]) {
    const GemmParams& p = *pp;
    const int tile_env = g_utx_opt.gemm_tile;
    if (!gemm_tile_known()) return -2;
    out[0] = 0; out[1] = ((p.M + 127) / 128) * ((p.N + 127) / 128); out[2] = 0; out[3] = 0;
    if (p.conv_Wo > 0 || p.mx8 == 1) return 0;
    if (p.mx8 != 2) {
        const bool ok256 = (p.N % 256 == 0) && (p.n_split >= p.N || p.n_split % 256 == 0) &&
                           (p.gelu_from >= p.N || p.gelu_from % 256 == 0) &&
                           (p.K2 == 0 || (p.lora_seg_n % 256 == 0 && p.lora_n_limit % 256 == 0));
        const long tiles256 = (long)((p.M + 255) / 256) * ((p.N + 255) / 256);
        if (!ok256 || tile_env == 128 || (tile_env == 0 && tiles256 < 192)) return 0;
        out[1] = (int)tiles256;
    } else {
        out[1] = ((p.M + 255) / 256) * (p.N / 256);
    }
    out[0] = 1;
    int grid = out[1] < ncu ? out[1] : ncu;
    if (g_utx_opt.gemm_pers_grid > 0 && g_utx_opt.gemm_pers_grid < grid) grid = g_utx_opt.gemm_pers_grid;
    utx_gemm_w4_split_plan(&p, out[1], grid, sk_has_work, &out[2], &out[3]);
    return 0;
}

extern "C" int utx_launch_gemm_bf16(const GemmParams* hp, hipStream_t stream) {
    GemmParams p = *hp;
    if (p.M <= 0 || p.N <= 0 || p.K <= 0) return -1;
    if (p.mx8) {
        if (!p.a_scale || !p.b_scale || (p.K % 128) || (p.lda & 15) || (p.ldb & 15) || p.conv_Wo > 0 || p.mx8 > 2) return -2;
        if (p.mx8 == 1 && ((p.lds_a & 3) || (p.lds_b & 3) || p.lds_a < p.K / 32 || p.lds_b < p.K / 32)) return -2;
        p.K /= 2; p.lda /= 2; p.ldb /= 2;
    }
    if ((p.K % GM_BK) || (p.K2 % GM_BK) || (p.N % 8)) return -2;
    if ((p.lda & 7) || (p.ldb & 7) || (p.ldc & 7)) return -2;
    if (p.K2 > 0 && (!p.A2 || !p.B2 || (p.lda2 & 7) || (p.ldb2 & 7) || p.lora_seg_n <= 0 || (p.lora_seg_n % 128))) return -2;
    if (p.gate && (!p.res || (p.ldres & 7))) return -2;
    if (p.n_split < p.N && (!p.C1 || (p.n_split % 128) || (p.ldc1 & 7))) return -2;
    const int group_env = g_utx_opt.gemm_group_m;
    if (!gemm_tile_known()) return -2;
    if (p.qk_cols > 0 && (p.mx8 || p.conv_Wo > 0 || p.gate)) return -2;
    if (p.q_out && p.mx8 != 2) return -2;
    if (p.conv_Wo > 0) {
        if (p.K2 > 0 || !p.zero_page || p.conv_cin_log2 < 6 || p.K != (9 << p.conv_cin_log2) || p.conv_Hi <= 0 || p.conv_Wi <= 0 ||
            p.conv_stride < 1 || p.conv_stride > 2 || p.conv_pad < 0 || p.conv_pad > 1 || (p.conv_up & ~1) || (p.M % p.conv_Wo))
            return -2;
        return launch_gemm<128, 128, 2, 2, true>(p, stream, 0);
    }
    if (p.mx8 == 2) {
        if ((p.N % 256) || (p.n_split < p.N && p.n_split % 256) || (p.gelu_from < p.N && p.gelu_from % 256) || p.K2 > 0 || p.qk_cols > 0) return -2;
        return utx_launch_gemm_w4(p, stream);
    }
    if (p.mx8) return launch_gemm<128, 128, 2, 2, false, true>(p, stream, group_env);
    int plan[4];
    (void)utx_gemm_plan_impl(&p, 256, 1, plan);
    if (p.qk_cols > 0) {
        if ((p.qk_cols % 256) || p.qk_cols > p.N || p.qk_cols > p.n_split || p.qk_cols > p.gelu_from ||
            !p.qk_wq || !p.qk_wk || !p.qk_cos || !p.qk_sin || !p.qk_Qh || !p.qk_Kh || p.qk_hs <= 0 || p.qk_tok_off < 0) return -2;
        if (plan[0] != 1) return -2;
    }
    if (plan[0] == 1) return utx_launch_gemm_w4(p, stream);
    return launch_gemm<128, 128, 2, 2>(p, stream, group_env);
}

extern "C" int utx_launch_gemv_bf16(const GemvParams* hp, hipStream_t stream) {
    GemvParams p = *hp;
    if (!p.x || !p.W || !p.y) return -2;
    if (p.M <= 0 || p.M > 8 || p.N <= 0 || p.K <= 0 || (p.K % 8) || (p.ldw & 7) || (p.ldx & 7)) return -2;
    if ((p.M > 1 && (p.ldx < p.K || p.ldy < p.N)) || (p.N > 1 && p.ldw < p.K)) return -2;
    hipLaunchKernelGGL(gemv_bf16_kernel, dim3((p.N + 3) / 4), dim3(256), 0, stream, p);
    return hipGetLastError() == hipSuccess ? 0 : -4;
}
```

### unitex_amd/csrc/kernels.h

```cpp
#pragma once
#include <hip/hip_runtime.h>
#include <stdint.h>
#include "../../include/unitex_hip.h"
#ifndef UTX_BF16_T
#define UTX_BF16_T
typedef uint16_t bf16_t;
#endif

struct AttnParams {
    const bf16_t* q;
    const bf16_t* k;
    const bf16_t* vt;
    bf16_t* o;
    long q_hs, q_ss, k_hs, k_ss, vt_hs, vt_ds, o_ss;
    int H, S, nqb;
    int Sq;
    int dbg;
    float scale_log2;
    unsigned char* flags;
    int flag_hs;
    int w_base, nsplit, tiles_per_split;
    bf16_t* part_o;
    float* part_lse;
    float key_bias_log2;
    int key_bias_period;
    void* work;
    size_t work_bytes;
    int blk_rows;
    long q_bs, k_bs, vt_bs;
};
struct Attn8Params {
    const uint8_t *q8, *k8;
    const uint8_t* v8t;
    const uint32_t *qs, *ks;
    const uint32_t* vs;
    bf16_t* o;
    long o_ss;
    int H, S, Sq, S_pad, nqb;
    float key_bias_log2;
    int key_bias_period;
    int w_base, nsplit, tiles_per_split;
    bf16_t* part_o;
    float* part_lse;
    void* work;
    size_t work_bytes;
};
struct UtxOptions {
    int attn_q64 = 1;
    int attn_tailsplit = 1;
    int gemm_group_m = 0;
    int gemm_tile = 0;
    int gemm_pers_grid = 0;
    int gemm_streamk = 1;
    int bvh_stack_walk = 0;
    int attn_var_abl = 0, attn_debug_abl = 0, gemm_debug_abl = 0;
    int bvh_packet = 1;
    int attn_peel = 1;
    int attn8_peel = 1;
    int gemm_fastk = 1;
    int nn_grid = 0;
};
extern UtxOptions g_utx_opt;

typedef utx_gemm_desc GemmParams;
typedef utx_knn_desc KnnParams;
typedef utx_gemv_desc GemvParams;
typedef utx_qkv_post_desc QkvPostParams;
typedef utx_ln_mod_desc LnModParams;
typedef utx_sched_desc SchedParams;

extern "C" {
int utx_launch_attn_fwd(const void* q, const void* k, const void* vt, void* o,
                        long q_hs, long q_ss, long k_hs, long k_ss, long vt_hs, long vt_ds,
                        long o_ss, int H, int S, int Sq, float scale, float key_bias_log2, int key_bias_period, void* work, size_t work_bytes, hipStream_t stream);
void utx_attn_split_plan_impl(int H, int Sq, int S, int ncu, int out[4]);
size_t utx_attn_workspace_bytes_impl(int H, int Sq, int S, int ncu);
size_t utx_attn_split_bytes_impl(int H, int Sq, int S, int ncu);
size_t utx_attn_q64_flag_bytes(int H, int Sq, int S);
int utx_attn_q64_takes(const AttnParams* p, int presc);
int utx_launch_attn_merge(const AttnParams* t, int n_items, hipStream_t stream);
int utx_launch_attn_fwd_glds(const AttnParams* p, int presc, hipStream_t stream);
int utx_launch_attn_fwd_fp8(const Attn8Params* p, hipStream_t stream);
int utx_launch_quant_vt_mx8(const void* vt, void* v8, void* vs, int H, int S_pad, hipStream_t stream);
int utx_launch_attn_fwd_blk(const void* q, const void* k, const void* vt, void* o, long q_hs, long q_ss, long k_hs, long k_ss, long vt_hs, long vt_ds,
                            long o_ss, int H, int S, int Sq, float scale, float key_bias_log2, int key_bias_period, void* work, size_t work_bytes,
                            int blk_rows, long q_bs, long k_bs, long vt_bs, hipStream_t stream);
int utx_launch_attn_fwd_q64(const AttnParams* p, int presc, hipStream_t stream);
int utx_launch_gemm_bf16(const GemmParams* p, hipStream_t stream);
size_t utx_gemm_streamk_workspace_bytes_impl(void);
int utx_gemm_plan_impl(const GemmParams* p, int ncu, int sk_has_work, int out[4]);
void utx_gemm_w4_split_plan(const GemmParams* p, int tiles, int grid, int has_work, int* T, int* S);
int utx_launch_gemm_w4(GemmParams p, hipStream_t stream);
int utx_launch_gemv_bf16(const GemvParams* p, hipStream_t stream);
int utx_launch_quant_mx8(const void* x, long ldx, void* q, long ldq, void* s, long lds, int M, int K, hipStream_t stream);
int utx_launch_quant_mx8_packed(const void* x, long ldx, void* q, long ldq, void* s, long row_blocks, int M, int K, hipStream_t stream);
int utx_launch_qkv_post(const QkvPostParams* p, hipStream_t stream);
int utx_launch_sp_unpack_qkv(const void* recv, int P, int Hp, int S_loc, int text_rows, void* q, void* k, void* vt, hipStream_t stream);
int utx_launch_sp_unpack_o(const void* recv, int P, int Hp, int S_loc, void* out, long ld, long src_cols, hipStream_t stream);
size_t utx_group_norm_workspace_bytes_impl(void);
int utx_launch_group_norm(const void* x, long npix, int C, const void* gamma, const void* beta, float eps, int silu, void* y, void* work, hipStream_t stream);
int utx_launch_softmax_rows(void* s, long nrow, long ld, int ncol, hipStream_t stream);
int utx_launch_conv3x3_thin(const void* x, int H, int W, int Cin, const void* wt, const void* bias, int Cout, void* y, hipStream_t stream);
int utx_launch_ln_mod(const LnModParams* p, hipStream_t stream);
int utx_launch_sched_step(const SchedParams* p, hipStream_t stream);
int utx_launch_transform(const float* verts, int V, const float* mvp, int n_views, float* clip, float* ndc, hipStream_t stream);
int utx_launch_rasterize(const float* pos, const int* tri, int F, int H, int W, float* rast, void* work, hipStream_t stream);
int utx_launch_interpolate(const float* attr, int C, const float* rast, const int* tri, long npix, float* out, hipStream_t stream);
int utx_launch_condition_shade(const float* rast, const float* nrm, const float* pos, const float* bg3_host, long npix, void* out_normal, void* out_ccm, void* out_alpha, hipStream_t stream);
int utx_launch_face_normals(const float* verts, const int* faces, int F, float* out, hipStream_t stream);
int utx_launch_view_visibility(const float* attr6, const float* rast, const float* fnormal, const float* dirs, const float* eyes, int n, int H, int W,
                               float grad_thr, float cos_thr, int radius, void* tmp, void* vis, float* alpha, hipStream_t stream);
size_t utx_knn_workspace_bytes_impl(long N);
int utx_launch_knn(const KnnParams* p, void* work, size_t work_bytes, hipStream_t stream);
size_t utx_fps_workspace_bytes_impl(long N);
int utx_launch_fps(const float* pos, const unsigned char* mask, long N, int M, int start, int* out_idx, float* out_d2, void* work, size_t work_bytes, hipStream_t stream);
int utx_launch_sample_edges(const float* verts, const int* edges, const int* edge_ids, const float* start, const float* length, int E, float total, long N,
                            float* samples, int* edge_index, float* edge_t, hipStream_t stream);
int utx_launch_sample_surface(const float* verts, const int* faces, const float* cum, int F, long N, unsigned long long seed, float* samples, int* face_index,
                              float* uvw, hipStream_t stream);
int utx_launch_texture_shade(const float* rast, const float* uv, const int* tri, const float* tex, int Ht, int Wt, const float* bg3_host, long npix, void* out, hipStream_t stream);
int utx_launch_gbuffer_shade(int mode, const float* rast, const int* tri, const float* attr, int stride, const float* scale2, int ndc, int composite, const float* bg3_host, long npix, void* out_u8, float* out_rgba, hipStream_t stream);
int utx_launch_gbuffer_range(int mode, const float* rast, const int* tri, const float* attr, int stride, long npix, float* scale2, int* empty, hipStream_t stream);
int utx_launch_camera_normals(const float* nrm, int V, const float* c2ws, int n_views, float* out, hipStream_t stream);
int utx_launch_uv_gbuffer(const float* rast, const int* tri, const float* v_pos, const float* v_nrm, const float* v_pos_cam, const float* v_nrm_cam, int V, int B, int H2D, int W2D,
                          unsigned want, void* const* outs_host, hipStream_t stream);
int utx_launch_screen_gbuffer(const float* rast, const int* tri, const float* v_pos, const float* v_nrm, const float* v_uv, const float* v_attr, int Ca, const float* clip_w,
                              const float* v_pos_cam, const float* v_nrm_cam, int V, int B, int H, int W, int n_maps, const float* const* maps_host, const int* map_dims_host,
                              int filter, int bg_kind, float bg_scalar, const float* bg_v_attr, const float* bg_map_attr, unsigned want, void* const* outs_host, hipStream_t stream);
int utx_launch_uv_project(const float* rast2d, const int* tri, int F, const unsigned char* face_mask, const float* v_ndc, int V, int B, int H2D, int W2D, const float* map,
                          int Bm, int Hm, int Wm, int C, const float* rast_map, int filter, int bg_kind, float bg_scalar, const float* bg, float* uv, float* uv_alpha,
                          float* map_attr, hipStream_t stream);
int utx_cubemap_table_impl(int N, float costheta_cutoff, float* texels_host, float* tiles_host);
int utx_launch_latlong_to_cubemap(const float* lat, int Hi, int Wi, int N, float* out, hipStream_t stream);
int utx_launch_cubemap_diffuse(const float* cube, int N, const float* texels, float* out, hipStream_t stream);
int utx_launch_cubemap_specular(const float* cube, int N, const float* texels, const float* tiles, float roughness, float costheta_cutoff, float* out, hipStream_t stream);
int utx_launch_dfg_lut(int R, int nsamples, float* out, hipStream_t stream);
int utx_launch_cube_sample(const float* cube, int N, const float* dirs, long n, float* out, hipStream_t stream);
int utx_launch_pbr_forward(const float* eye, int eye_stride, const float* pos, const float* nrm, const float* kd, int kd_stride, const float* ks, const float* light_diffuse, int Nd,
                           const float* light_specular, int Ns, const float* lut, int R, long npix, float* out_diffuse, float* out_specular, hipStream_t stream);
int utx_launch_pbr_shade(const float* rast, const int* tri, const float* vpos, const float* vnrm, const float* vuv, const float* kd, int Hk, int Wk, const float* ks, int Hs, int Ws,
                         const float* eye3_host, const float* light_diffuse, int Nd, const float* light_specular, int Ns, const float* lut, int R, float lambda_diffuse,
                         float lambda_specular, const float* bg3_host, long npix, void* out_u8, float* out_rgba, hipStream_t stream);
int utx_launch_pbr_shading_normal(const float* eye, int eye_stride, const float* pos, const float* pert, const float* snrm, const float* stng, const float* gnrm, long npix,
                                  float* out, hipStream_t stream);
int utx_launch_pbr_shade_nm(const float* rast, const int* tri, const float* vpos, const float* vnrm, const float* vtng, const float* fnrm, const float* vuv, const float* kd, int Hk,
                            int Wk, const float* ks, int Hs, int Ws, const float* nm, int Hn, int Wn, const float* eye3_host, const float* light_diffuse, int Nd,
                            const float* light_specular, int Ns, const float* lut, int R, float lambda_diffuse, float lambda_specular, const float* bg3_host, long npix,
                            void* out_u8, float* out_rgba, hipStream_t stream);
int utx_bvh_build_impl(const float* verts, int V, const int* faces, int F, utx_bvh** out, hipStream_t stream);
size_t utx_bvh_workspace_bytes_impl(int F);
int utx_bvh_build_ws_impl(const float* verts, int V, const int* faces, int F, void* work, size_t work_bytes, utx_bvh** out, hipStream_t stream);
void utx_bvh_free_impl(utx_bvh* b);
int utx_bvh_arrays_impl(utx_bvh* b, int** info, float** aabb, unsigned** codes_sorted, int** idx_sorted);
int utx_bvh_trace_impl(utx_bvh* b, const float* ro, const float* rd, long R, int* tid, unsigned long long* visited, int force_stack, hipStream_t stream);
int utx_bvh_depth_impl(utx_bvh* b);
int utx_visible_faces_rays_impl(utx_bvh* b, const float* verts, const int* faces, int F, const float* c2ws, int B, int perspective, int flags, unsigned char* mask,
                                unsigned long long* visited, hipStream_t stream);
int utx_launch_visible_faces_raster(const float* rast, int B, int H, int W, int F, unsigned char* mask, hipStream_t stream);
int utx_launch_erode_faces(unsigned char* mask, const int* faces, int B, int F, int V, int depth, int* vstamp, hipStream_t stream);
int utx_launch_visible_vertices(const unsigned char* mask, const int* faces, int B, int F, int V, unsigned char* out, hipStream_t stream);
int utx_launch_view_weight_maps(const float* cosn, const float* cam_nrm, int B, int H, int W, int r, void* tmp, float* out, float* arccos_out, hipStream_t stream);
int utx_launch_vertex_project(const float* v_pos, int V, const unsigned char* visible, int B, const float* xform, const float* proj, const float* images, int Hi, int Wi,
                              const float* wmap, int H, int W, const float* v_rgb, const float* weights, int use_alpha, float* acc, float* wacc, float overlay_conf,
                              int blending, float blending_conf, float inpainting_conf, float* blended, unsigned char* inpaint, hipStream_t stream);
int utx_launch_vertex_inpaint_step(const int* rowptr, const int* col, const int* idx, int n, const float* rgb_in, const unsigned char* mask_in, float* rgb_out,
                                   unsigned char* mask_out, int* counter, hipStream_t stream);
int utx_launch_uv_bake(const float* rast2d, const int* faces, int F, const unsigned char* face_mask, const float* v_ndc, int V, int B, int Th, int Tw,
                       const float* images, const float* wmap, const float* rast_view, int R, const float* map_Kd, const float* weights, int use_alpha,
                       float* acc, float* wacc, float overlay_conf, int blending, float blending_conf, float inpainting_conf, float* blended,
                       unsigned char* inpaint, hipStream_t stream);
int utx_launch_uv_dilation_step(const float* col_in, const unsigned char* mask_in, int H, int W, int C, int mode, float* col_out, unsigned char* mask_out,
                                int* counter, hipStream_t stream);
int utx_launch_backproject(const utx_backproject_desc* p, const float* eyes, int sample, const utx_bvh* bvh, hipStream_t stream);
int utx_launch_backproject_vis(const utx_backproject_desc* p, const float* eyes, int sample, const utx_bvh* bvh, hipStream_t stream);
int utx_launch_composite_winner(const void* vis, int n_views, const int* order, int n_order, long T, void* winner, hipStream_t stream);
int utx_launch_gather_winner(const float* rast2d, const int* faces, const float* vndc, const float* images, const void* winner, long T, int V, int n_views, int H, int W, int C, int sample, float* atlas, hipStream_t stream);
// ... 14 lines not shown
```

### unitex_amd/csrc/plan.cpp

```cpp
#include <hip/hip_runtime.h>
#include <string.h>
#include <vector>
#include "kernels.h"

namespace {
enum Kind { K_GEMM, K_GEMV, K_LN_MOD, K_QKV_POST, K_ATTN, K_QUANT, K_ADD3, K_FORK, K_JOIN, K_QUANT_VT, K_ATTN8 };
struct AttnArgs { const void *q, *k, *vt; void* o; long q_hs, q_ss, k_hs, k_ss, vt_hs, vt_ds, o_ss; int H, S_q, S_kv; float scale, kb; int period; void* work; size_t work_bytes; };
struct QuantArgs { const void* x; long ldx; void* q; long ldq; void* s; long lds; int M, K, packed; };
struct Add3Args { const void *a, *b, *c; void* out; int n; };
struct QuantVtArgs { const void* vt; void *v8, *vs; int H, S_pad; };
struct Entry {
    Kind kind; int side;
    union { utx_gemm_desc gemm; utx_gemv_desc gemv; utx_ln_mod_desc ln; utx_qkv_post_desc qkv; AttnArgs attn; QuantArgs quant; Add3Args add3; QuantVtArgs qvt; Attn8Params attn8; };
    Entry() { memset(this, 0, sizeof(*this)); }
};
}

struct utx_plan {
    std::vector<Entry> entries;
    hipStream_t side = nullptr;
    std::vector<hipEvent_t> events;
    int cur_side = 0, open_sections = 0;
    int device = 0;
};
// ... 20 lines not shown

int utx_plan_size(const utx_plan* p) { return p ? (int)p->entries.size() : -2; }

static Entry& push(utx_plan* p, Kind k) { p->entries.emplace_back(); Entry& e = p->entries.back(); e.kind = k; e.side = p->cur_side; return e; }

int utx_plan_add_gemm(utx_plan* p, const utx_gemm_desc* d) { if (!p || !d) return -2; push(p, K_GEMM).gemm = *d; return 0; }
int utx_plan_add_gemv(utx_plan* p, const utx_gemv_desc* d) { if (!p || !d) return -2; push(p, K_GEMV).gemv = *d; return 0; }
int utx_plan_add_ln_mod(utx_plan* p, const utx_ln_mod_desc* d) { if (!p || !d) return -2; push(p, K_LN_MOD).ln = *d; return 0; }
int utx_plan_add_qkv_post(utx_plan* p, const utx_qkv_post_desc* d) { if (!p || !d) return -2; push(p, K_QKV_POST).qkv = *d; return 0; }
int utx_plan_add_attn(utx_plan* p, const void* q, const void* k, const void* vt, void* o, long q_hs, long q_ss, long k_hs, long k_ss, long vt_hs,
                      long vt_ds, long o_ss, int H, int S_q, int S_kv, float softmax_scale, float key_bias_log2, int key_bias_period, void* work,
                      size_t work_bytes) {
    if (!p || !q || !k || !vt || !o) return -2;
    AttnArgs a = {q, k, vt, o, q_hs, q_ss, k_hs, k_ss, vt_hs, vt_ds, o_ss, H, S_q, S_kv, softmax_scale, key_bias_log2, key_bias_period, work, work_bytes};
    push(p, K_ATTN).attn = a;
    return 0;
}
int utx_plan_add_quant_mx8(utx_plan* p, const void* x, long ldx, void* q, long ldq, void* s, long lds_or_row_blocks, int M, int K, int packed) {
    if (!p || !x || !q || !s) return -2;
    QuantArgs a = {x, ldx, q, ldq, s, lds_or_row_blocks, M, K, packed};
    push(p, K_QUANT).quant = a;
    return 0;
}
int utx_plan_add_add3(utx_plan* p, const void* a, const void* b, const void* c, void* out, int n) {
    if (!p || !a || !c || !out || n <= 0) return -2;
    Add3Args g = {a, b, c, out, n};
    push(p, K_ADD3).add3 = g;
    return 0;
}
int utx_plan_add_quant_vt_mx8(utx_plan* p, const void* vt, void* v8, void* vs, int H, int S_pad) {
    if (!p || !vt || !v8 || !vs) return -2;
    QuantVtArgs a = {vt, v8, vs, H, S_pad};
    push(p, K_QUANT_VT).qvt = a;
    return 0;
}
int utx_plan_add_attn_fp8(utx_plan* p, const void* q8, const void* qs, const void* k8, const void* ks, const void* v8t, const void* vs, void* o, long o_ss,
                          int H, int S_q, int S_kv, int S_pad, float key_bias_log2, int key_bias_period) {
    if (!p || !q8 || !qs || !k8 || !ks || !v8t || !vs || !o) return -2;
    Attn8Params a;
    memset(&a, 0, sizeof(a));
    a.q8 = (const uint8_t*)q8; a.k8 = (const uint8_t*)k8; a.v8t = (const uint8_t*)v8t;
    a.qs = (const uint32_t*)qs; a.ks = (const uint32_t*)ks; a.vs = (const uint32_t*)vs;
    a.o = (bf16_t*)o; a.o_ss = o_ss; a.H = H; a.S = S_kv; a.Sq = S_q; a.S_pad = S_pad;
    a.key_bias_log2 = key_bias_log2; a.key_bias_period = key_bias_period;
    push(p, K_ATTN8).attn8 = a;
    return 0;
}
int utx_plan_add_attn_fp8_ws(utx_plan* p, const void* q8, const void* qs, const void* k8, const void* ks, const void* v8t, const void* vs, void* o, long o_ss,
                             int H, int S_q, int S_kv, int S_pad, float key_bias_log2, int key_bias_period, void* work, size_t work_bytes) {
    const int rc = utx_plan_add_attn_fp8(p, q8, qs, k8, ks, v8t, vs, o, o_ss, H, S_q, S_kv, S_pad, key_bias_log2, key_bias_period);
    if (rc) return rc;
    p->entries.back().attn8.work = work;
    p->entries.back().attn8.work_bytes = work ? work_bytes : 0;
    return 0;
}
int utx_plan_fork(utx_plan* p) {
    if (!p || p->cur_side || p->open_sections) return -2;
    if (!p->side && hipStreamCreateWithFlags(&p->side, hipStreamNonBlocking) != hipSuccess) return -5;
    hipEvent_t a, b;
    if (hipEventCreateWithFlags(&a, hipEventDisableTiming) != hipSuccess) return -5;
    if (hipEventCreateWithFlags(&b, hipEventDisableTiming) != hipSuccess) { (void)hipEventDestroy(a); return -5; }
    p->events.push_back(a); p->events.push_back(b);
    push(p, K_FORK);
    p->cur_side = 1; p->open_sections = 1;
    return 0;
}
int utx_plan_main(utx_plan* p) { if (!p || !p->open_sections) return -2; p->cur_side = 0; return 0; }
int utx_plan_join(utx_plan* p) {
    if (!p || !p->open_sections) return -2;
    p->cur_side = 0; p->open_sections = 0;
    push(p, K_JOIN);
    return 0;
}

int utx_plan_assign_sk(utx_plan* p, void* sk_work, size_t sk_work_bytes, int n_cus) {
    if (!p || !sk_work || n_cus <= 0) return 0;
    bool any = false;
    for (const Entry& e : p->entries)
        if (e.kind == K_GEMM && !e.side && (long)((e.gemm.M + 255) / 256) * (e.gemm.N / 256) > n_cus) any = true;
    if (!any) return 0;
    int n = 0;
    for (Entry& e : p->entries)
        if (e.kind == K_GEMM && !e.side) { e.gemm.sk_work = sk_work; e.gemm.sk_work_bytes = sk_work_bytes; ++n; }
    return n;
}

int utx_plan_entry(const utx_plan* p, int i, int* kind, int* side, void* buf, size_t cap) {
    if (!p || i < 0 || i >= (int)p->entries.size() || !kind || !side) return -2;
    const Entry& e = p->entries[i];
    *kind = (int)e.kind; *side = e.side;
    const void* src = nullptr; size_t n = 0;
    switch (e.kind) {
        case K_GEMM: src = &e.gemm; n = sizeof(e.gemm); break;
        case K_GEMV: src = &e.gemv; n = sizeof(e.gemv); break;
        case K_LN_MOD: src = &e.ln; n = sizeof(e.ln); break;
        case K_QKV_POST: src = &e.qkv; n = sizeof(e.qkv); break;
        case K_ATTN: src = &e.attn; n = sizeof(e.attn); break;
        case K_QUANT: src = &e.quant; n = sizeof(e.quant); break;
        case K_ADD3: src = &e.add3; n = sizeof(e.add3); break;
        case K_QUANT_VT: src = &e.qvt; n = sizeof(e.qvt); break;
        case K_ATTN8: src = &e.attn8; n = sizeof(e.attn8); break;
        default: break;
    }
    if (n > cap) return -2;
    if (n && buf) memcpy(buf, src, n);
    return (int)n;
}

int utx_plan_run_range(utx_plan* p, int begin, int end, utx_stream stream_, int* failed_entry) {
    if (!p || p->open_sections || begin < 0 || end > (int)p->entries.size() || begin > end) return -2;
    hipStream_t main_s = (hipStream_t)stream_;
    size_t section = 0;
    int open_at_begin = 0;
    for (int i = 0; i < begin; ++i) {
        if (p->entries[i].kind == K_FORK) ++open_at_begin;
        if (p->entries[i].kind == K_JOIN) { ++section; --open_at_begin; }
    }
    if (open_at_begin != 0) { if (failed_entry) *failed_entry = begin; return -2; }
    bool forked = false;
    int rc = 0, bad = -1;
    for (int i = begin; i < end; ++i) {
        const Entry& e = p->entries[i];
        hipStream_t st = e.side ? p->side : main_s;
        if ((e.side || e.kind == K_JOIN) && !forked) { rc = -2; bad = i; break; }
        switch (e.kind) {
            case K_GEMM: rc = utx_launch_gemm_bf16(&e.gemm, st); break;
            case K_GEMV: rc = utx_launch_gemv_bf16(&e.gemv, st); break;
            case K_LN_MOD: rc = utx_launch_ln_mod(&e.ln, st); break;
            case K_QKV_POST: rc = utx_launch_qkv_post(&e.qkv, st); break;
            case K_ATTN: {
                const AttnArgs& a = e.attn;
                rc = utx_launch_attn_fwd(a.q, a.k, a.vt, a.o, a.q_hs, a.q_ss, a.k_hs, a.k_ss, a.vt_hs, a.vt_ds, a.o_ss, a.H, a.S_kv, a.S_q, a.scale, a.kb,
                                         a.period, a.work, a.work_bytes, st);
                break;
            }
            case K_QUANT: {
                const QuantArgs& a = e.quant;
                rc = a.packed ? utx_launch_quant_mx8_packed(a.x, a.ldx, a.q, a.ldq, a.s, a.lds, a.M, a.K, st)
                              : utx_launch_quant_mx8(a.x, a.ldx, a.q, a.ldq, a.s, a.lds, a.M, a.K, st);
                break;
            }
            case K_ADD3: rc = utx_launch_add3_bf16(e.add3.a, e.add3.b, e.add3.c, e.add3.out, e.add3.n, st); break;
            case K_QUANT_VT: rc = utx_launch_quant_vt_mx8(e.qvt.vt, e.qvt.v8, e.qvt.vs, e.qvt.H, e.qvt.S_pad, st); break;
            case K_ATTN8: rc = utx_launch_attn_fwd_fp8(&e.attn8, st); break;
            case K_FORK:
                if (hipEventRecord(p->events[2 * section], main_s) != hipSuccess || hipStreamWaitEvent(p->side, p->events[2 * section], 0) != hipSuccess) rc = -4;
                else forked = true;
                break;
            case K_JOIN:
                if (hipEventRecord(p->events[2 * section + 1], p->side) != hipSuccess || hipStreamWaitEvent(main_s, p->events[2 * section + 1], 0) != hipSuccess) rc = -4;
                forked = false;
                ++section;
                break;
        }
        if (rc != 0) { bad = i; break; }
    }
    if (rc == 0 && forked) { rc = -2; bad = end; }
    if (forked) {
        if (hipEventRecord(p->events[2 * section + 1], p->side) == hipSuccess) (void)hipStreamWaitEvent(main_s, p->events[2 * section + 1], 0);
    }
    if (rc != 0 && failed_entry) *failed_entry = bad;
    return rc;
}

int utx_plan_run(utx_plan* p, utx_stream stream_, int* failed_entry) {
    if (!p) return -2;
// ... 5 lines not shown
```

### unitex_amd/flux/ops.py

```python
import ctypes as C
import math

import torch

from .. import _lib
from .._lib import GemmDesc, GemvDesc, LnModDesc, QkvPostDesc, SchedDesc, ptr

_CTX = {}


def get_ctx(device=None):
    if device is None:
        device = torch.cuda.current_device()
    if device not in _CTX:
        _CTX[device] = _lib.Context(device)
    return _CTX[device]


def _bf(t):
    assert t.is_cuda and t.dtype == torch.bfloat16, "expected a CUDA bf16 tensor"
    return t


def attention(q, k, vt, S=None, scale=None, out=None, o_ss=None, key_bias_log2=0.0, key_bias_period=0, S_q=None):
# ... 29 lines not shown
    ctx = get_ctx(vt.device.index)
    H, D, S_pad = vt.shape
    assert D == 128 and S_pad % 64 == 0 and vt.is_contiguous()
    v8, vs = out if out is not None else (torch.empty(H, 128, S_pad, dtype=torch.uint8, device=vt.device), torch.empty(H, S_pad // 32, 32, 4, dtype=torch.uint8, device=vt.device))
    ctx.check(ctx.lib.utx_quant_vt_mx8(ctx.handle, ptr(vt), ptr(v8), ptr(vs), H, S_pad, ctx.stream()))
    return v8, vs


def attention_fp8(q8, qs, k8, ks, v8t, vs, S=None, S_q=None, out=None, o_ss=None, key_bias_log2=0.0, key_bias_period=0):
    ctx = get_ctx(q8.device.index)
    H, S_pad, D = q8.shape
    assert D == 128 and v8t.shape == (H, 128, S_pad)
    S = S_pad if S is None else S
    S_q = S if S_q is None else S_q
    if out is None:
        out = torch.empty(S_q, H * 128, dtype=torch.bfloat16, device=q8.device)
    if o_ss is None:
        o_ss = out.stride(0)
    ctx.check(ctx.lib.utx_attn_fwd_fp8(ctx.handle, ptr(q8), ptr(qs), ptr(k8), ptr(ks), ptr(v8t), ptr(vs), ptr(out), o_ss, H, S_q, S, S_pad,
                                       float(key_bias_log2), int(key_bias_period), ctx.stream()))
    return out


def make_gemm_desc(A, B, C_out, bias=None, A2=None, B2=None, lora_n_limit=None, lora_seg_n=None, alpha=1.0,
                   gelu_from=None, gate=None, res=None, n_split=None, C1=None, a_scale=None, b_scale=None, qk_post=None, sk_work=None, q_out=None):
    M, K = A.shape
    N = B.shape[0]
    d = GemmDesc()
    d.A, d.lda, d.B, d.ldb = ptr(A), A.stride(0), ptr(B), B.stride(0)
    if a_scale is not None:
        assert A.dtype == torch.uint8 and B.dtype == torch.uint8 and b_scale is not None
        if hasattr(a_scale, "row_blocks"):
            assert hasattr(b_scale, "row_blocks"), "packed activation scales need packed weight scales"
            d.a_scale, d.lds_a, d.b_scale, d.lds_b, d.mx8 = ptr(a_scale.data), a_scale.row_blocks, ptr(b_scale.data), b_scale.row_blocks, 2
        else:
            d.a_scale, d.lds_a, d.b_scale, d.lds_b, d.mx8 = ptr(a_scale), a_scale.stride(0), ptr(b_scale), b_scale.stride(0), 1
    if A2 is not None:
        d.A2, d.lda2, d.B2, d.ldb2 = ptr(A2), A2.stride(0), ptr(B2), B2.stride(0)
        d.K2 = B2.shape[1]
        d.lora_n_limit = N if lora_n_limit is None else lora_n_limit
        d.lora_seg_n = N if lora_seg_n is None else lora_seg_n
    else:
        d.K2, d.lora_n_limit, d.lora_seg_n = 0, 0, 128
    d.M, d.N, d.K = M, N, K
    if qk_post is not None:
        q = qk_post
        d.qk_cols, d.qk_tok_off, d.qk_eps, d.qk_q_scale = int(q["cols"]), int(q["tok_off"]), float(q["eps"]), float(q["q_scale"])
        d.qk_wq, d.qk_wk, d.qk_cos, d.qk_sin = ptr(q["wq"]), ptr(q["wk"]), ptr(q["cos"]), ptr(q["sin"])
        d.qk_Qh, d.qk_Kh, d.qk_hs = ptr(q["Qh"]), ptr(q["Kh"]), q["Qh"].stride(0)
    d.alpha = alpha
    d.bias = ptr(bias)
    d.gelu_from = N if gelu_from is None else gelu_from
    d.gate = ptr(gate)
    if gate is not None:
        d.res, d.ldres = ptr(res), res.stride(0)
    d.C, d.ldc = ptr(C_out), C_out.stride(0)
    d.n_split = N if n_split is None else n_split
    if C1 is not None:
        d.C1, d.ldc1 = ptr(C1), C1.stride(0)
    if sk_work is not None:
        d.sk_work, d.sk_work_bytes = ptr(sk_work), sk_work.numel() * sk_work.element_size()
    if q_out is not None:
        qv, qs, kt0 = q_out
        d.q_out, d.ldq_out, d.qs_out, d.qs_out_rb, d.q_out_kt0 = ptr(qv), qv.stride(0), ptr(qs), qs.stride(0) // 512, int(kt0)
    return d


_SK_WS = {}


def streamk_workspace(device, stream=None, shared=True):
    dev = torch.device(device)
    ctx = get_ctx(dev.index)
    nbytes = int(ctx.lib.utx_gemm_streamk_workspace_bytes(ctx.handle))
    if not shared:
        return torch.empty(nbytes, dtype=torch.uint8, device=dev)
    st = torch.cuda.current_stream(dev) if stream is None else stream
    key = (dev.index, st.cuda_stream)
    if key not in _SK_WS:
        _SK_WS[key] = torch.empty(nbytes, dtype=torch.uint8, device=dev)
    return _SK_WS[key]


GEMM_KERNELS = ("128x128", "w4")


def gemm_plan(M, N, K=3072, K2=0, n_split=None, gelu_from=None, lora_seg_n=None, lora_n_limit=None, sk=True, n_cus=256):
    lib = _lib.load_library()
    d = GemmDesc()
    d.A = d.B = d.C = 1
    d.M, d.N, d.K, d.K2 = int(M), int(N), int(K), int(K2)
    d.lora_n_limit = (N if lora_n_limit is None else lora_n_limit) if K2 else 0
    d.lora_seg_n = (N if lora_seg_n is None else lora_seg_n) if K2 else 128
    d.n_split = N if n_split is None else n_split
    d.gelu_from = N if gelu_from is None else gelu_from
    d.sk_work = 1 if sk else None
    out = (C.c_int * 4)()
    rc = lib.utx_gemm_plan(C.byref(d), int(n_cus), C.byref(out))
    if rc != 0:
        raise ValueError("utx_gemm_plan -> %d" % rc)
    return {"kernel": GEMM_KERNELS[out[0]], "tiles": out[1], "tail_tiles": out[2], "ranges": out[3]}


def gemm_takes_w4(M, N, n_split=None, gelu_from=None, K2=0, lora_seg_n=None, lora_n_limit=None):
    return gemm_plan(M, N, K2=K2, n_split=n_split, gelu_from=gelu_from, lora_seg_n=lora_seg_n, lora_n_limit=lora_n_limit)["kernel"] == "w4"


def mx8_uses_packed(M, N, n_split=None, gelu_from=None):
    if N % 256 or (n_split is not None and n_split < N and n_split % 256) or (gelu_from is not None and gelu_from < N and gelu_from % 256):
        return False
    return ((M + 255) // 256) * (N // 256) >= 192


def gemm(A, B, bias=None, out=None, **kw):
    ctx = get_ctx(A.device.index)
    M, N = A.shape[0], B.shape[0]
    n_split = kw.get("n_split")
    if out is None:
        out = torch.empty(M, N if n_split is None else n_split, dtype=torch.bfloat16, device=A.device)
    if kw.get("a_scale") is None:
        _bf(A), _bf(B)
    if "sk_work" not in kw and M >= 4096:
        kw = dict(kw, sk_work=streamk_workspace(A.device))
    d = make_gemm_desc(A, B, out, bias=bias, **kw)
    ctx.check(ctx.lib.utx_gemm_bf16(ctx.handle, C.byref(d), ctx.stream()))
    return out


def gemv(x, W, bias=None, silu_in=False, silu_out=False, out=None):
    ctx = get_ctx(x.device.index)
    M, K = x.shape
    N = W.shape[0]
    if out is None:
        out = torch.empty(M, N, dtype=torch.bfloat16, device=x.device)
    d = GemvDesc()
    d.x, d.ldx, d.W, d.ldw, d.bias = ptr(_bf(x)), x.stride(0), ptr(_bf(W)), W.stride(0), ptr(bias)
    d.y, d.ldy, d.M, d.N, d.K = ptr(out), out.stride(0), M, N, K
    d.silu_in, d.silu_out = int(silu_in), int(silu_out)
    ctx.check(ctx.lib.utx_gemv_bf16(ctx.handle, C.byref(d), ctx.stream()))
    return out


def qkv_post(qkv, q_col, k_col, v_col, wq, wk, cos, sin, Qh, Kh, Vt, n_tok, tok_off, H, eps=1e-6, q_scale=1.0,
             heads_per_group=0, group_stride=0, head_stride=None, row_stride_v=None, skip_qk=False, sub_heads=0, sub_stride=0):
    ctx = get_ctx(qkv.device.index)
    d = QkvPostDesc()
    d.qkv, d.ld = ptr(_bf(qkv)), qkv.stride(0)
    d.q_col, d.k_col, d.v_col = q_col, k_col, v_col
    d.wq, d.wk = ptr(_bf(wq)), ptr(_bf(wk))
    assert cos.dtype == torch.float32 and sin.dtype == torch.float32 and cos.is_contiguous()
    d.cosb, d.sinb = ptr(cos), ptr(sin)
    d.Qh, d.Kh, d.Vt = ptr(Qh), ptr(Kh), ptr(Vt)
    if heads_per_group:
        d.hs_qk, d.hs_v, d.S_pad = head_stride, head_stride, row_stride_v
        d.heads_per_group, d.gs_qk, d.gs_v = heads_per_group, group_stride, group_stride
        d.sub_heads, d.gs2_qk, d.gs2_v = sub_heads, sub_stride, sub_stride
    else:
        d.hs_qk, d.hs_v, d.S_pad = Qh.stride(0), Vt.stride(0), Vt.shape[2]
    d.n_tok, d.tok_off, d.H, d.eps, d.q_scale = n_tok, tok_off, H, eps, q_scale
    d.skip_qk = int(bool(skip_qk))
    ctx.check(ctx.lib.utx_qkv_post(ctx.handle, C.byref(d), ctx.stream()))


def ln_mod(x, shift, scale, out=None, eps=1e-6):
    ctx = get_ctx(x.device.index)
    if out is None:
        out = torch.empty_like(x)
# ... 17 lines not shown
```

### unitex_amd/flux/transformer.py

```python
import ctypes as C
import math
import os
from typing import Dict, List, Optional, Tuple

import torch

from .._lib import GemvDesc, LnModDesc, QkvPostDesc, ptr
from . import ops

BF16 = torch.bfloat16

LORA_TARGETS_DOUBLE = ["attn.to_q", "attn.to_k", "attn.to_v", "attn.to_out.0", "attn.add_q_proj",
                       "attn.add_k_proj", "attn.add_v_proj", "attn.to_add_out", "ff.net.0.proj", "ff.net.2",
                       "ff_context.net.0.proj", "ff_context.net.2"]


class FluxShape:

    def __init__(self, num_heads=24, num_double=19, num_single=38, in_channels=64, joint_dim=4096,
                 pooled_dim=768, axes_dim=(16, 56, 56), theta=10000.0, mlp_ratio=4, guidance_embeds=True):
        self.num_heads, self.head_dim = num_heads, 128
        self.num_double, self.num_single = num_double, num_single
        self.in_channels, self.joint_dim, self.pooled_dim = in_channels, joint_dim, pooled_dim
        self.axes_dim, self.theta, self.mlp_ratio = tuple(axes_dim), theta, mlp_ratio
# ... 552 lines not shown
                    a_o = PackedScales(ws["asp2"], n_out, Kmax)
                    plan.append(("quant_mx8", (cat[r0:r1], ws["aq2"], a_o)))
                    plan.append((self.lib.utx_gemm_bf16, ops.make_gemm_desc(ws["aq2"], b["out.q"], h[r0:r1], bias=b["out.b"], gate=g_, res=h[r0:r1],
                                                                            a_scale=a_o, b_scale=b["out.sp"])))
                    continue
                lora = b.get("lora.qkvm")
                kw_kv, kw_q = {}, {}
                if lora is not None:
                    A_cat, B_cat, alpha, _rp = lora
                    R = A_cat.shape[0] // 3
                    Tv = T[:S, : 3 * R]
                    plan.append((self.lib.utx_gemm_bf16, ops.make_gemm_desc(xn, A_cat, Tv, alpha=alpha)))
                    kw_kv = dict(A2=Tv[:, R:], B2=B_cat[D: 3 * D], lora_n_limit=2 * D, lora_seg_n=D)
                    kw_q = dict(A2=Tv[r0:r1, :R], B2=B_cat[:D], lora_n_limit=D, lora_seg_n=D)
                plan.append((self.lib.utx_gemm_bf16, ops.make_gemm_desc(xn, Wm[D: 3 * D], qkv[:, D: 3 * D], bias=bm[D: 3 * D], **kw_kv)))
                plan.append((self.lib.utx_gemm_bf16, ops.make_gemm_desc(xn[r0:r1], Wm[:D], qkv[r0:r1, :D], bias=bm[:D], **kw_q)))
                plan.append((self.lib.utx_gemm_bf16, ops.make_gemm_desc(xn[r0:r1], Wm[3 * D:], cat[r0:r1, D:], bias=bm[3 * D:], gelu_from=0)))
                self._qkvpost(plan, qkv, b["nq"], b["nk"], ws, S, 0)
                self._attn(plan, ws, cat[r0:], S, q_rows=(r0, r1))
                plan.append((self.lib.utx_gemm_bf16, ops.make_gemm_desc(cat[r0:r1], b["out.w"], h[r0:r1], bias=b["out.b"], gate=g_, res=h[r0:r1])))
                continue
            if self.sp is None:
                has_l = b.get("lora.qkvm") is not None
                qkm = qk_fused(S, (3 + sh.mlp_ratio) * D, 0, b["nq"], b["nk"], n_split=3 * D, gelu_from=3 * D, K2=(Rp if has_l else 0),
                               lora_seg_n=D, lora_n_limit=3 * D)
                self._gemm(plan, xn, b["qkvm.w"], qkv, bias=b["qkvm.b"], lora=b.get("lora.qkvm"), lora_n_limit=3 * D,
                           lora_seg_n=D, T=T, gelu_from=3 * D, n_split=3 * D, C1=cat[:, D:], mx8=m_qkvm, qk_post=qkm)
                self._qkvpost(plan, qkv, b["nq"], b["nk"], ws, S, 0, skip_qk=qkm is not None)
            else:
                if sp_mx is not None:
                    Wq, Wsp = sp_mx
                    NW = Wq.shape[0]
                    m_a = (Wq[: 3 * D], Wsp.row_slice(0, 3 * D), ws["aq"], ws["asp"], {"quant_cols": 0 if f_sgl else D})
                    m_b = (Wq[3 * D:], Wsp.row_slice(3 * D, NW), ws["aq"], ws["asp"],
                           dict({"quant_cols": 0}, **({"q_out": (ws["aq"][:S, D:], ws["asp"], D // 128)} if f_sgl else {})))
                else:
                    m_a = m_b = None
                self._gemm(plan, xn, b["qkvm.w"][: 3 * D], qkv, bias=b["qkvm.b"][: 3 * D], lora=b.get("lora.qkvm"),
                           lora_n_limit=3 * D, lora_seg_n=D, T=T, mx8=m_a)
                self._qkvpost(plan, qkv, b["nq"], b["nk"], ws, S, 0)
                plan.append(("sp_start", None))
                self._gemm(plan, xn, b["qkvm.w"][3 * D:], cat[:, D:], bias=b["qkvm.b"][3 * D:], gelu_from=0, mx8=m_b)
            self._attn(plan, ws, cat, S)
            self._gemm(plan, cat, b["out.w"], h, bias=b["out.b"], gate=g_, res=h, mx8=m_out)
        o = self.mod_off[("out",)]
        scale, shift = mod[o: o + D], mod[o + D: o + 2 * D]
        self._lnmod(plan, h_x[:n_out], xn_x[:n_out], shift, scale)
        self._gemm(plan, xn_x[:n_out], W["proj_out.w"], ws["out"][:n_out], bias=W["proj_out.b"])
        self._assign_streamk(plan, ws)
        return {"ws": ws, "plan": plan, "S_txt": S_txt, "S_img": S_img, "n_out": n_out}

    def gemm_census(self, n_cus=None):
        if not self._plans:
            return {}
        if n_cus is None:
            n_cus = torch.cuda.get_device_properties(self.device).multi_processor_count
        out = {}
        arr = (C.c_int * 4)()

        def walk(entries):
            for e in entries:
                if e[0] == "par":
                    walk(e[1][0]); walk(e[1][1])
                elif e[0] is self.lib.utx_gemm_bf16:
                    if self.lib.utx_gemm_plan(C.byref(e[1]), int(n_cus), C.byref(arr)) != 0:
                        continue
                    k = ops.GEMM_KERNELS[arr[0]]
                    out[k] = out.get(k, 0) + 1
                    if arr[2] > 0:
                        out["w4_split_tail"] = out.get("w4_split_tail", 0) + 1
        walk(next(iter(self._plans.values()))["plan"])
        return out

    def _assign_streamk(self, plan, ws):
        ncu = torch.cuda.get_device_properties(self.device).multi_processor_count

        def main_gemms(entries):
            for e in entries:
                if e[0] is self.lib.utx_gemm_bf16:
                    yield e[1]
                elif e[0] == "par":
                    yield from main_gemms(e[1][0])
        descs = list(main_gemms(plan))
        if not any(((d.M + 255) // 256) * (d.N // 256) > ncu for d in descs):
            return
        if "sk" not in ws:
            ws["sk"] = ops.streamk_workspace(self.device, shared=False)
        sk = ws["sk"]
        for d in descs:
            d.sk_work, d.sk_work_bytes = ptr(sk), sk.numel()

    TEXT_KEEP = 64

    def local_text_range(self, S_txt):
        from .ulysses import local_slice
        return (0, S_txt) if self.sp is None else local_slice(S_txt, self.sp[0], self.sp[1])

    def local_image_range(self, S_img):
        from .ulysses import local_slice
        return (0, S_img) if self.sp is None else local_slice(S_img, self.sp[0], self.sp[1])

    def __del__(self):
        try:
            self._drop_plans()
        except Exception:
            pass

    def _drop_plans(self):
        for p in self._plans.values():
            if p.get("cplan") is not None:
                self.lib.utx_plan_free(p["cplan"])
                p["cplan"] = None
        self._plans.clear()
        self._graphs = {}

    def _tproj_device(self, t1000):
        c = self.__dict__.setdefault("_tproj_cache", {})
        t = c.get(t1000)
        if t is None:
            if len(c) > 4096:
                c.clear()
            t = c[t1000] = _timestep_proj(t1000).to(self.device)
        return t

    def set_output_rows(self, n):
        self.out_rows = None if n is None else int(n)

    def set_positions(self, txt_ids, img_ids):
        self._ids = (txt_ids.detach().to("cpu", torch.float32).contiguous(), img_ids.detach().to("cpu", torch.float32).contiguous())
        self.out_rows = None

    def set_conditioning(self, encoder_hidden_states, pooled_projections, guidance: float):
        if self._ids is None:
            raise RuntimeError("set_positions must be called before set_conditioning")
        txt_ids, img_ids = self._ids
        S_txt = encoder_hidden_states.shape[-2]
        assert txt_ids.shape[0] == S_txt, "txt_ids and encoder_hidden_states disagree on the number of text tokens"
        enc = encoder_hidden_states.reshape(S_txt, -1)
        world = 1 if self.sp is None else self.sp[1]
        K = self.TEXT_KEEP
        identical = bool(self.text_dedup and S_txt > K * world and S_txt % (K * world) == 0 and
                         torch.equal(txt_ids, txt_ids[:1].expand_as(txt_ids)) and torch.equal(enc, enc[:1].expand_as(enc)))
        self.sp_kv_dedup = bool(identical and world > 1 and not self.fp8_attention and os.environ.get("UTX_SP_ZERO_COPY", "0") != "1" and
                                os.environ.get("UTX_SP_KV_DEDUP", "1") != "0")
        if identical:
            t0, t1 = 0, K
            self.key_bias_log2 = math.log2(S_txt / float(K * (1 if self.sp_kv_dedup else world)))
            self.text_rows = K
        else:
            t0, t1 = self.local_text_range(S_txt)
            self.key_bias_log2, self.text_rows = 0.0, None
        i0, i1 = self.local_image_range(img_ids.shape[0])
        S_loc = (t1 - t0) + (i1 - i0)
        self.key_bias_period = (S_loc // 64) if (identical and world > 1 and not self.sp_kv_dedup) else 0
        key = (t1 - t0, i1 - i0, self._lora_version, self.key_bias_log2, self.key_bias_period, self.out_rows, self.sp_kv_dedup)
        if key not in self._plans:
            self._drop_plans()
            self._plans[key] = self._build(t1 - t0, i1 - i0)
            if os.environ.get("UTX_C_PLAN", "1") != "0":
                self.compile_plan(self._plans[key])
        p = self._plans[key]
        ws = p["ws"]
        cos, sin = rope_tables(torch.cat([txt_ids[t0:t1], img_ids[i0:i1]], dim=0), self.shape.axes_dim, self.shape.theta)
        ws["cos"].copy_(cos, non_blocking=True)
        ws["sin"].copy_(sin, non_blocking=True)
        ws["enc"].copy_(enc[t0:t1].to(BF16))
        ws["pooled"].copy_(pooled_projections.reshape(1, -1).to(BF16))
        g1000 = _bf16_scalar(_bf16_scalar(guidance) * 1000.0)
        ws["gproj"].copy_(_timestep_proj(g1000))

    def _launch(self, fn, d, st, timed=True):
        gev = self.gemm_events
        if gev is not None and timed and fn is self.lib.utx_gemm_bf16 and d.M >= 4096:
# ... 181 lines not shown
        if not ok:
            lib.utx_plan_free(h)
            return None
        if segments is not None:
            segments.append((seg_begin, int(lib.utx_plan_size(h)), None))
        old = p.get("cplan")
        if old is not None:
            lib.utx_plan_free(old)
        p["cplan"] = h
        p["segments"] = segments
        return h

    def _run_segments(self, p):
        st, ws = self.ctx.stream(), p["ws"]
        bad = C.c_int(-1)
        for b0, b1, host_op in p["segments"]:
            if b1 > b0:
                rc = self.lib.utx_plan_run_range(p["cplan"], b0, b1, st, C.byref(bad))
                if rc:
                    raise RuntimeError("utx_plan_run_range [%d, %d): entry %d failed with code %d" % (b0, b1, bad.value, rc))
            if host_op is not None:
                self._sp_entry(host_op[0], host_op[1], ws, st)

    def build_c_dit_plan(self, p=None):
        from .._lib import DitConfig, DitDoubleBlock, DitLinear, DitSingleBlock, DitWeights, DitWorkspace
        if self.sp is not None or self.fuse_qk or self.fp8_attention:
            return None
        p = next(iter(self._plans.values())) if p is None else p
        ws, sh, W = p["ws"], self.shape, self.W

        def lin(w, b_, lora=None, blk=None, nm=None):
            L = DitLinear()
            L.w, L.b = ptr(w), ptr(b_)
            if lora is not None:
                A_cat, B_cat, alpha, Rp = lora
                L.lora_A, L.lora_B, L.lora_alpha, L.lora_rp, L.lora_nseg = ptr(A_cat), ptr(B_cat), float(alpha), int(Rp), A_cat.shape[0] // Rp
            if self.fp8_weights and blk is not None and (nm + ".q") in blk:
                L.q, L.s, L.lds_s = ptr(blk[nm + ".q"]), ptr(blk[nm + ".s"]), blk[nm + ".s"].stride(0)
                sp = blk.get(nm + ".sp")
                if sp is not None:
                    L.sp, L.sp_row_blocks = ptr(sp.data), sp.row_blocks
            return L
        wt = DitWeights()
        wt.x_embedder = lin(self._w("x_embedder.w"), self._w("x_embedder.b"))
        wt.context_embedder = lin(W["context_embedder.w"], W["context_embedder.b"])
        wt.proj_out = lin(W["proj_out.w"], W["proj_out.b"])
        k = "time_text_embed.%s.%s"
        for dst, nm in (("t", "timestep_embedder"), ("g", "guidance_embedder"), ("p", "text_embedder")):
            if nm == "guidance_embedder" and not sh.guidance_embeds:
                continue
            for j in (1, 2):
                setattr(wt, "%s_lin%d" % (dst, j), lin(W[k % (nm, "linear_%d" % j) + ".w"], W[k % (nm, "linear_%d" % j) + ".b"]))
        wt.mod = lin(W["mod.w"], W["mod.b"])
        dbl = (DitDoubleBlock * max(1, len(self.double)))()
        for i, b in enumerate(self.double):
            for nm in ("qkv_x", "qkv_c", "out_x", "out_c", "ff1_x", "ff2_x", "ff1_c", "ff2_c"):
                setattr(dbl[i], nm, lin(b[nm + ".w"], b[nm + ".b"], b.get("lora." + nm), b, nm))
            dbl[i].nq, dbl[i].nk, dbl[i].naq, dbl[i].nak = ptr(b["nq"]), ptr(b["nk"]), ptr(b["naq"]), ptr(b["nak"])
            dbl[i].mod_x, dbl[i].mod_c = self.mod_off[("d", i, "x")], self.mod_off[("d", i, "c")]
        sgl = (DitSingleBlock * max(1, len(self.single)))()
        for i, b in enumerate(self.single):
            sgl[i].qkvm = lin(b["qkvm.w"], b["qkvm.b"], b.get("lora.qkvm"), b, "qkvm")
            sgl[i].out = lin(b["out.w"], b["out.b"], None, b, "out")
            sgl[i].nq, sgl[i].nk, sgl[i].mod = ptr(b["nq"]), ptr(b["nk"]), self.mod_off[("s", i)]
        wt.dbl, wt.sgl = dbl, sgl
        wt.mod_out, wt.n_mod = self.mod_off[("out",)], self.n_mod
        cfg = DitConfig()
        cfg.num_heads, cfg.num_double, cfg.num_single = sh.num_heads, sh.num_double, sh.num_single
        cfg.in_channels, cfg.joint_dim, cfg.pooled_dim, cfg.mlp_ratio, cfg.guidance_embeds = sh.in_channels, sh.joint_dim, sh.pooled_dim, sh.mlp_ratio, int(sh.guidance_embeds)
        cfg.S_txt, cfg.S_img, cfg.n_out = p["S_txt"], p["S_img"], p["n_out"]
        cfg.key_bias_log2, cfg.key_bias_period = float(self.key_bias_log2), int(self.key_bias_period)
        cfg.two_streams = int(bool(self.overlap_text))
        cfg.n_cus = torch.cuda.get_device_properties(self.device).multi_processor_count
        cfg.lora_rank_padded = int(self.lora_rank) if self._lora_active else 0
        cfg.fp8 = int(bool(self.fp8_weights))
        cfg.fp8_fuse_quant = int(bool(self.fp8_weights) and os.environ.get("UTX_FP8_FUSE_QUANT", "1") != "0")
        w = DitWorkspace()
        for nm in ("lat", "enc", "pooled", "tproj", "gproj", "e1", "e_t", "e_g", "e_p", "temb", "mod", "h", "xn", "qkv", "cat", "attn", "out", "cos", "sin", "Qh", "Kh",
                   "Vt", "T", "Tc"):
            setattr(w, nm, ptr(ws.get(nm)))
        sk, aw = ws.get("sk"), ws.get("attn_ws")
        w.sk_work, w.sk_work_bytes = ptr(sk), 0 if sk is None else sk.numel()
        w.attn_work, w.attn_work_bytes = ptr(aw), 0 if aw is None else aw.numel()
        if self.fp8_weights:
            w.aq, w.as_rm, w.asp, w.asp_row_blocks = ptr(ws["aq"]), ptr(ws["as"]), ptr(ws["asp"]), ws["asp"].stride(0) // 512
            if "aq2" in ws:
                w.aq2, w.asp2, w.asp2_row_blocks = ptr(ws["aq2"]), ptr(ws["asp2"]), ws["asp2"].stride(0) // 512
        h = C.c_void_p()
        self.ctx.check(self.lib.utx_dit_load(self.ctx.handle, C.byref(cfg), C.byref(wt), C.byref(w), C.byref(h)))
        return h

    def forward(self, hidden_states, timestep: float, out: Optional[torch.Tensor] = None):
        p = next(iter(self._plans.values()))
        ws = p["ws"]
        t1000 = _bf16_scalar(_bf16_scalar(timestep) * 1000.0)
        ws["tproj"].copy_(self._tproj_device(t1000), non_blocking=True)
        if hidden_states.data_ptr() != ws["lat"].data_ptr():
            ws["lat"].copy_(hidden_states.reshape(ws["lat"].shape))
        g = self._graphs.get(id(p))
        if g is not None:
            g.replay()
        elif p.get("cplan") is not None and self.attn_events is None and self.gemm_events is None:
            if p.get("segments") is not None:
                self._run_segments(p)
            else:
                bad = C.c_int(-1)
                rc = self.lib.utx_plan_run(p["cplan"], self.ctx.stream(), C.byref(bad))
                if rc:
                    raise RuntimeError("utx_plan_run: entry %d failed with code %d" % (bad.value, rc))
        else:
            self.run_plan(p)
        if out is not None:
            out.copy_(ws["out"])
            return out
        return ws["out"]

    def capture_graph(self, warm=True):
        p = next(iter(self._plans.values()))
        if getattr(self, "attn_events", None) is not None:
            raise RuntimeError("per-kernel event timing and graph replay are exclusive")
        if warm:
            self.run_plan(p)
        torch.cuda.synchronize(self.device)
        g = torch.cuda.CUDAGraph()
        with torch.cuda.graph(g):
            self.run_plan(p)
        self._graphs = {id(p): g}
        return g

    def release_graph(self):
        self._graphs = {}

    __call__ = forward
```

Baseline: 0.5756.

## Add split-K skinny GEMM kernel for small-M text-stream linears

Adds a dedicated GEMM path for M<=64 (text tokens) that tiles N by 64 and splits K across ranges so that enough workgroups exist to fill the CUs. Each range writes fp32 partials to a workspace, and a fixup kernel reduces them and applies the bias/GELU/gate epilogue. This targets under-occupancy of the 128x128 tile kernel on skinny text-stream GEMMs. In exchange it adds a second launch per GEMM, a dedicated workspace allocation, and a reduction pass through global memory. It is skipped for fp8 weights.

```diff
diff --git a/include/unitex_hip.h b/include/unitex_hip.h
--- a/include/unitex_hip.h
+++ b/include/unitex_hip.h
@@ -83,6 +83,7 @@
 } utx_gemm_desc;
 int utx_gemm_bf16(utx_ctx* ctx, const utx_gemm_desc* d, utx_stream stream);
 size_t utx_gemm_streamk_workspace_bytes(utx_ctx* ctx);
+size_t utx_gemm_skinny_workspace_bytes(const utx_gemm_desc* d, int n_cus);
 int utx_gemm_plan(const utx_gemm_desc* d, int n_cus, int out[4]);
 
 int utx_quant_mx8(utx_ctx* ctx, const void* x, long ldx, void* q, long ldq, void* s, long lds, int M, int K, utx_stream stream);
@@ -402,6 +403,7 @@
 int utx_plan_run(utx_plan* plan, utx_stream stream, int* failed_entry);
 int utx_plan_run_range(utx_plan* plan, int begin, int end, utx_stream stream, int* failed_entry);
 int utx_plan_assign_sk(utx_plan* plan, void* sk_work, size_t sk_work_bytes, int n_cus);
+int utx_plan_assign_sk_txt(utx_plan* plan, void* work, size_t work_bytes);
 int utx_plan_entry(const utx_plan* plan, int i, int* kind, int* side, void* buf, size_t cap);
 
 typedef struct utx_dit_linear {
@@ -440,6 +442,7 @@
     void* attn_work; size_t attn_work_bytes;
     void *aq, *as_rm, *asp; int asp_row_blocks;
     void *aq2, *asp2; int asp2_row_blocks;
+    void* sk_txt_work; size_t sk_txt_work_bytes;
 } utx_dit_workspace;
 int utx_dit_load(utx_ctx* ctx, const utx_dit_config* cfg, const utx_dit_weights* weights, const utx_dit_workspace* ws, utx_plan** out);
 int utx_dit_step(utx_plan* plan, utx_stream stream, int* failed_entry);
diff --git a/unitex_amd/_lib.py b/unitex_amd/_lib.py
--- a/unitex_amd/_lib.py
+++ b/unitex_amd/_lib.py
@@ -96,7 +96,8 @@
     _fields_ = [(n, c_void_p) for n in ("lat", "enc", "pooled", "tproj", "gproj", "e1", "e_t", "e_g", "e_p", "temb", "mod", "h", "xn", "qkv", "cat", "attn", "out",
                                         "cos", "sin", "Qh", "Kh", "Vt", "T", "Tc")] + \
                [("sk_work", c_void_p), ("sk_work_bytes", C.c_size_t), ("attn_work", c_void_p), ("attn_work_bytes", C.c_size_t),
-                ("aq", c_void_p), ("as_rm", c_void_p), ("asp", c_void_p), ("asp_row_blocks", c_int), ("aq2", c_void_p), ("asp2", c_void_p), ("asp2_row_blocks", c_int)]
+                ("aq", c_void_p), ("as_rm", c_void_p), ("asp", c_void_p), ("asp_row_blocks", c_int), ("aq2", c_void_p), ("asp2", c_void_p), ("asp2_row_blocks", c_int),
+                ("sk_txt_work", c_void_p), ("sk_txt_work_bytes", C.c_size_t)]
 
 
 ABI_STRUCTS = [GemmDesc, GemvDesc, QkvPostDesc, LnModDesc, SchedDesc, BackprojectDesc, KnnDesc, DitLinear, DitDoubleBlock, DitSingleBlock, DitWeights, DitConfig,
@@ -127,6 +128,7 @@
     "utx_plan_run": (c_int, [c_void_p, c_void_p, C.POINTER(c_int)]),
     "utx_plan_run_range": (c_int, [c_void_p, c_int, c_int, c_void_p, C.POINTER(c_int)]),
     "utx_plan_assign_sk": (c_int, [c_void_p, c_void_p, C.c_size_t, c_int]),
+    "utx_plan_assign_sk_txt": (c_int, [c_void_p, c_void_p, C.c_size_t]),
     "utx_plan_entry": (c_int, [c_void_p, c_int, C.POINTER(c_int), C.POINTER(c_int), c_void_p, C.c_size_t]),
     "utx_dit_load": (c_int, [c_void_p, C.POINTER(DitConfig), C.POINTER(DitWeights), C.POINTER(DitWorkspace), C.POINTER(c_void_p)]),
     "utx_dit_step": (c_int, [c_void_p, c_void_p, C.POINTER(c_int)]),
@@ -147,6 +149,7 @@
     "utx_attn_plan": (c_int, [c_int, c_int, c_int, c_int, c_void_p]),
     "utx_gemm_bf16": (c_int, [c_void_p, C.POINTER(GemmDesc), c_void_p]),
     "utx_gemm_streamk_workspace_bytes": (C.c_size_t, [c_void_p]),
+    "utx_gemm_skinny_workspace_bytes": (C.c_size_t, [C.POINTER(GemmDesc), c_int]),
     "utx_gemm_plan": (c_int, [C.POINTER(GemmDesc), c_int, C.POINTER(c_int * 4)]),
     "utx_quant_mx8": (c_int, [c_void_p, c_void_p, c_long, c_void_p, c_long, c_void_p, c_long, c_int, c_int, c_void_p]),
     "utx_quant_mx8_packed": (c_int, [c_void_p, c_void_p, c_long, c_void_p, c_long, c_void_p, c_long, c_int, c_int, c_void_p]),
diff --git a/unitex_amd/csrc/build.py b/unitex_amd/csrc/build.py
--- a/unitex_amd/csrc/build.py
+++ b/unitex_amd/csrc/build.py
@@ -18,6 +18,7 @@
     ("attention_fp8.hip", NO_PK),
     ("gemm.hip", []),
     ("gemm_w4.hip", []),
+    ("gemm_skinny.hip", []),
     ("dit_elementwise.hip", ["-ffp-contract=off"] + NO_PK),
     ("vae.hip", NO_PK),
     ("capi.cpp", []),
diff --git a/unitex_amd/csrc/capi.cpp b/unitex_amd/csrc/capi.cpp
--- a/unitex_amd/csrc/capi.cpp
+++ b/unitex_amd/csrc/capi.cpp
@@ -244,6 +244,7 @@
 }
 
 size_t utx_gemm_streamk_workspace_bytes(utx_ctx*) { return utx_gemm_streamk_workspace_bytes_impl(); }
+size_t utx_gemm_skinny_workspace_bytes(const utx_gemm_desc* d, int n_cus) { return (d && n_cus > 0) ? utx_gemm_skinny_workspace_bytes_impl(d, n_cus) : 0; }
 int utx_gemm_plan(const utx_gemm_desc* d, int n_cus, int out[4]) {
     if (!d || !out || n_cus <= 0 || d->M <= 0 || d->N <= 0 || d->K <= 0) return -2;
     options_from_env_once();
diff --git a/unitex_amd/csrc/common.h b/unitex_amd/csrc/common.h
--- a/unitex_amd/csrc/common.h
+++ b/unitex_amd/csrc/common.h
@@ -26,6 +26,12 @@
     return __builtin_bit_cast(uint32_t, v);
 }
 __device__ __forceinline__ float rbf(float f) { return bf2f(f2bf(f)); }
+
+__device__ __forceinline__ float gelu_tanh(float x) {
+    const float k0 = 0.7978845608028654f, k1 = 0.044715f;
+    const float u = k0 * (x + k1 * x * x * x);
+    return x * __builtin_amdgcn_rcpf(1.0f + __expf(-2.0f * u));
+}
 
 __device__ __forceinline__ float wave_sum(float v) {
 #pragma unroll
diff --git a/unitex_amd/csrc/dit_plan.cpp b/unitex_amd/csrc/dit_plan.cpp
--- a/unitex_amd/csrc/dit_plan.cpp
+++ b/unitex_amd/csrc/dit_plan.cpp
@@ -6,6 +6,7 @@
 
 extern "C" {
 int utx_plan_assign_sk(utx_plan* p, void* sk_work, size_t sk_work_bytes, int n_cus);
+int utx_plan_assign_sk_txt(utx_plan* p, void* work, size_t work_bytes);
 }
 
 namespace {
@@ -277,6 +278,7 @@
     b.linear(wt->proj_out, xn_x, D, n_out, D, c.in_channels, ws->out, c.in_channels, true, nullptr, 0, 0);
     if (b.rc) { utx_plan_free(plan); return b.rc; }
     utx_plan_assign_sk(plan, ws->sk_work, ws->sk_work_bytes, ncu);
+    utx_plan_assign_sk_txt(plan, ws->sk_txt_work, ws->sk_txt_work_bytes);
     *out = plan;
     return 0;
 }
diff --git a/unitex_amd/csrc/gemm.hip b/unitex_amd/csrc/gemm.hip
--- a/unitex_amd/csrc/gemm.hip
+++ b/unitex_amd/csrc/gemm.hip
@@ -1,15 +1,10 @@
 #include "common.h"
 #include "kernels.h"
+#include "gemm_skinny_plan.h"
 #include <stdlib.h>
 
 #define GM_BK 64
 #define GM_GROUP_M 4
-
-__device__ __forceinline__ float gelu_tanh(float x) {
-    const float k0 = 0.7978845608028654f, k1 = 0.044715f;
-    const float u = k0 * (x + k1 * x * x * x);
-    return x * __builtin_amdgcn_rcpf(1.0f + __expf(-2.0f * u));
-}
 
 __device__ __forceinline__ void glds16(const bf16_t* g, char* lds) {
     __builtin_amdgcn_global_load_lds((const __attribute__((address_space(1))) void*)g,
@@ -329,7 +324,7 @@
 
 static bool gemm_tile_known() {
     const int t = g_utx_opt.gemm_tile;
-    return t == 0 || t == 128 || t == 2564;
+    return t == 0 || t == 64 || t == 128 || t == 2564;
 }
 
 extern "C" int utx_gemm_plan_impl(const GemmParams* pp, int ncu, int sk_has_work, int out[4]) {
@@ -338,12 +333,17 @@
     if (!gemm_tile_known()) return -2;
     out[0] = 0; out[1] = ((p.M + 127) / 128) * ((p.N + 127) / 128); out[2] = 0; out[3] = 0;
     if (p.conv_Wo > 0 || p.mx8 == 1) return 0;
+    if (p.M <= 64 && utx_gemm_skinny_takes(&p, ncu)) {
+        const SknPlan s = skn_plan(p.N, p.K, ncu);
+        out[0] = 5; out[1] = s.nchunks; out[3] = s.ranges;
+        return 0;
+    }
     if (p.mx8 != 2) {
         const bool ok256 = (p.N % 256 == 0) && (p.n_split >= p.N || p.n_split % 256 == 0) &&
                            (p.gelu_from >= p.N || p.gelu_from % 256 == 0) &&
                            (p.K2 == 0 || (p.lora_seg_n % 256 == 0 && p.lora_n_limit % 256 == 0));
         const long tiles256 = (long)((p.M + 255) / 256) * ((p.N + 255) / 256);
-        if (!ok256 || tile_env == 128 || (tile_env == 0 && tiles256 < 192)) return 0;
+        if (!ok256 || tile_env == 128 || ((tile_env == 0 || tile_env == 64) && tiles256 < 192)) return 0;
         out[1] = (int)tiles256;
     } else {
         out[1] = ((p.M + 255) / 256) * (p.N / 256);
@@ -365,7 +365,9 @@
     }
     if ((p.K % GM_BK) || (p.K2 % GM_BK) || (p.N % 8)) return -2;
     if ((p.lda & 7) || (p.ldb & 7) || (p.ldc & 7)) return -2;
-    if (p.K2 > 0 && (!p.A2 || !p.B2 || (p.lda2 & 7) || (p.ldb2 & 7) || p.lora_seg_n <= 0 || (p.lora_seg_n % 128))) return -2;
+    const int skinny_ncu = (p.M <= 64 && !p.mx8 && p.conv_Wo == 0) ? utx_ncu() : 0;
+    const bool skinny = skinny_ncu > 0 && utx_gemm_skinny_takes(&p, skinny_ncu);
+    if (p.K2 > 0 && (!p.A2 || !p.B2 || (p.lda2 & 7) || (p.ldb2 & 7) || p.lora_seg_n <= 0 || (p.lora_seg_n % (skinny ? 64 : 128)))) return -2;
     if (p.gate && (!p.res || (p.ldres & 7))) return -2;
     if (p.n_split < p.N && (!p.C1 || (p.n_split % 128) || (p.ldc1 & 7))) return -2;
     const int group_env = g_utx_opt.gemm_group_m;
@@ -383,6 +385,7 @@
         return utx_launch_gemm_w4(p, stream);
     }
     if (p.mx8) return launch_gemm<128, 128, 2, 2, false, true>(p, stream, group_env);
+    if (skinny) return utx_launch_gemm_skinny(p, skinny_ncu, stream);
     int plan[4];
     (void)utx_gemm_plan_impl(&p, 256, 1, plan);
     if (p.qk_cols > 0) {
diff --git a/unitex_amd/csrc/gemm_skinny.hip b/unitex_amd/csrc/gemm_skinny.hip
--- /dev/null
+++ b/unitex_amd/csrc/gemm_skinny.hip
@@ -0,0 +1,178 @@
+#include "common.h"
+#include "kernels.h"
+#include "gemm_skinny_plan.h"
+
+typedef __attribute__((ext_vector_type(4))) float skn_f32x4;
+
+struct SknFrag { bf16x8 b[2][4]; bf16x8 a[2][4]; };
+
+__device__ __forceinline__ void skn_load(SknFrag& f, const bf16_t* b0, const bf16_t* b1, const bf16_t* a0, const bf16_t* a1) {
+#pragma unroll
+    for (int kk = 0; kk < 4; ++kk) {
+        f.b[0][kk] = *reinterpret_cast<const bf16x8*>(b0 + 16 * kk);
+        f.b[1][kk] = *reinterpret_cast<const bf16x8*>(b1 + 16 * kk);
+        f.a[0][kk] = *reinterpret_cast<const bf16x8*>(a0 + 16 * kk);
+        f.a[1][kk] = *reinterpret_cast<const bf16x8*>(a1 + 16 * kk);
+    }
+}
+
+__global__ __launch_bounds__(256, 2) void gemm_skinny_kernel(GemmParams p, int nchunks, int ranges, int tiles_per_range) {
+    __shared__ skn_f32x4 red[3][16][64];
+    const int tid = threadIdx.x, lane = tid & 63;
+    const int wave = __builtin_amdgcn_readfirstlane(tid >> 6);
+    const int l31 = lane & 31, lh = lane >> 5;
+    const int chunk = blockIdx.x % nchunks, r = blockIdx.x / nchunks;
+    const int n0 = chunk * SKN_BN;
+    const int nk1 = p.K / SKN_BK;
+    const int t0 = r * tiles_per_range;
+    const int t1 = (t0 + tiles_per_range < nk1) ? t0 + tiles_per_range : nk1;
+    const bool lora = (r == ranges - 1) && (p.K2 > 0) && ((n0 & ~127) < p.lora_n_limit);
+    const int nmain = t1 - t0;
+    const int nt = nmain + (lora ? p.K2 / SKN_BK : 0);
+    const long a2_off = lora ? (long)(n0 / p.lora_seg_n) * p.K2 : 0;
+    const int i0 = (wave * nt) / 4, i1 = ((wave + 1) * nt) / 4;
+
+    const int nb0 = (n0 + l31 > p.N - 1) ? p.N - 1 : n0 + l31;
+    const int nb1 = (n0 + 32 + l31 > p.N - 1) ? p.N - 1 : n0 + 32 + l31;
+    const int ma0 = (l31 > p.M - 1) ? p.M - 1 : l31;
+    const int ma1 = (32 + l31 > p.M - 1) ? p.M - 1 : 32 + l31;
+    const bf16_t* const pb0 = (const bf16_t*)p.B + (long)nb0 * p.ldb + 8 * lh + (long)t0 * SKN_BK;
+    const bf16_t* const pb1 = (const bf16_t*)p.B + (long)nb1 * p.ldb + 8 * lh + (long)t0 * SKN_BK;
+    const bf16_t* const pa0 = (const bf16_t*)p.A + (long)ma0 * p.lda + 8 * lh + (long)t0 * SKN_BK;
+    const bf16_t* const pa1 = (const bf16_t*)p.A + (long)ma1 * p.lda + 8 * lh + (long)t0 * SKN_BK;
+    const bf16_t* const qb0 = lora ? (const bf16_t*)p.B2 + (long)nb0 * p.ldb2 + 8 * lh - (long)nmain * SKN_BK : pb0;
+    const bf16_t* const qb1 = lora ? (const bf16_t*)p.B2 + (long)nb1 * p.ldb2 + 8 * lh - (long)nmain * SKN_BK : pb1;
+    const bf16_t* const qa0 = lora ? (const bf16_t*)p.A2 + a2_off + (long)ma0 * p.lda2 + 8 * lh - (long)nmain * SKN_BK : pa0;
+    const bf16_t* const qa1 = lora ? (const bf16_t*)p.A2 + a2_off + (long)ma1 * p.lda2 + 8 * lh - (long)nmain * SKN_BK : pa1;
+#define SKN_LOAD(f_, i_)                                                                                      \
+    {                                                                                                         \
+        const bool main_ = (i_) < nmain;                                                                      \
+        const long ko_ = (long)(i_) * SKN_BK;                                                                 \
+        skn_load(f_, (main_ ? pb0 : qb0) + ko_, (main_ ? pb1 : qb1) + ko_, (main_ ? pa0 : qa0) + ko_, (main_ ? pa1 : qa1) + ko_); \
+    }
+
+    f32x16 acc[2][2];
+#pragma unroll
+    for (int a = 0; a < 2; ++a)
+#pragma unroll
+        for (int b = 0; b < 2; ++b)
+#pragma unroll
+            for (int q = 0; q < 16; ++q) acc[a][b][q] = 0.f;
+
+#define SKN_MFMA(f_)                                                                                          \
+    _Pragma("unroll") for (int kk = 0; kk < 4; ++kk)                                                          \
+        _Pragma("unroll") for (int ni = 0; ni < 2; ++ni)                                                      \
+            _Pragma("unroll") for (int mi = 0; mi < 2; ++mi)                                                  \
+                acc[ni][mi] = __builtin_amdgcn_mfma_f32_32x32x16_bf16(f_.b[ni][kk], f_.a[mi][kk], acc[ni][mi], 0, 0, 0);
+    if (i0 < i1) {
+        SknFrag f0, f1;
+        SKN_LOAD(f0, i0)
+        for (int i = i0; i < i1; i += 2) {
+            const int ia = (i + 1 < i1) ? i + 1 : i1 - 1;
+            SKN_LOAD(f1, ia)
+            __builtin_amdgcn_sched_barrier(0);
+            SKN_MFMA(f0)
+            __builtin_amdgcn_sched_barrier(0);
+            const int ib = (i + 2 < i1) ? i + 2 : i1 - 1;
+            SKN_LOAD(f0, ib)
+            __builtin_amdgcn_sched_barrier(0);
+            if (i + 1 < i1) { SKN_MFMA(f1) }
+            __builtin_amdgcn_sched_barrier(0);
+        }
+    }
+
+    if (wave > 0) {
+#pragma unroll
+        for (int ni = 0; ni < 2; ++ni)
+#pragma unroll
+            for (int mi = 0; mi < 2; ++mi)
+#pragma unroll
+                for (int a = 0; a < 4; ++a)
+                    red[wave - 1][(ni * 2 + mi) * 4 + a][lane] =
+                        skn_f32x4{acc[ni][mi][4 * a], acc[ni][mi][4 * a + 1], acc[ni][mi][4 * a + 2], acc[ni][mi][4 * a + 3]};
+    }
+    __syncthreads();
+    if (wave == 0) {
+        skn_f32x4* const dst = (skn_f32x4*)p.sk_work + ((long)r * nchunks + chunk) * (16 * 64) + lane;
+#pragma unroll
+        for (int ni = 0; ni < 2; ++ni)
+#pragma unroll
+            for (int mi = 0; mi < 2; ++mi)
+#pragma unroll
+                for (int a = 0; a < 4; ++a) {
+                    const int q = (ni * 2 + mi) * 4 + a;
+                    skn_f32x4 v = skn_f32x4{acc[ni][mi][4 * a], acc[ni][mi][4 * a + 1], acc[ni][mi][4 * a + 2], acc[ni][mi][4 * a + 3]};
+                    v += red[0][q][lane];
+                    v += red[1][q][lane];
+                    v += red[2][q][lane];
+                    dst[q * 64] = v;
+                }
+    }
+}
+
+__device__ __forceinline__ void skn_epilogue(const GemmParams& p, int m, int n, skn_f32x4 acc) {
+    float bv[4] = {0.f, 0.f, 0.f, 0.f};
+    if (p.bias) {
+        const uint2 braw = *reinterpret_cast<const uint2*>((const bf16_t*)p.bias + n);
+        bv[0] = bf2f((uint16_t)(braw.x & 0xffff)); bv[1] = bf2f((uint16_t)(braw.x >> 16));
+        bv[2] = bf2f((uint16_t)(braw.y & 0xffff)); bv[3] = bf2f((uint16_t)(braw.y >> 16));
+    }
+    const bool do_gelu = n >= p.gelu_from;
+    float y[4];
+#pragma unroll
+    for (int c = 0; c < 4; ++c) {
+        float v = rbf(acc[c] * p.alpha + bv[c]);
+        if (do_gelu) v = gelu_tanh(v);
+        y[c] = v;
+    }
+    uint32_t o[2] = {pack2bf(y[0], y[1]), pack2bf(y[2], y[3])};
+    if (p.gate) {
+        const uint2 rr = *reinterpret_cast<const uint2*>((const bf16_t*)p.res + (long)m * p.ldres + n);
+        const uint2 gg = *reinterpret_cast<const uint2*>((const bf16_t*)p.gate + n);
+        const uint32_t rw[2] = {rr.x, rr.y}, gw[2] = {gg.x, gg.y};
+#pragma unroll
+        for (int c = 0; c < 2; ++c) {
+            const float y0 = bf2f((uint16_t)(o[c] & 0xffff)), y1 = bf2f((uint16_t)(o[c] >> 16));
+            const float r0 = bf2f((uint16_t)(rw[c] & 0xffff)), r1 = bf2f((uint16_t)(rw[c] >> 16));
+            const float g0 = bf2f((uint16_t)(gw[c] & 0xffff)), g1 = bf2f((uint16_t)(gw[c] >> 16));
+            o[c] = pack2bf(r0 + rbf(g0 * y0), r1 + rbf(g1 * y1));
+        }
+    }
+    bf16_t* const dst = (n >= p.n_split) ? (bf16_t*)p.C1 + (long)m * p.ldc1 + (n - p.n_split) : (bf16_t*)p.C + (long)m * p.ldc + n;
+    *reinterpret_cast<uint2*>(dst) = make_uint2(o[0], o[1]);
+}
+
+__global__ __launch_bounds__(256) void gemm_skinny_fixup_kernel(GemmParams p, int nchunks, int ranges) {
+    const int chunk = blockIdx.x >> 2;
+    const int q = (blockIdx.x & 3) * 4 + (threadIdx.x >> 6);
+    const int lane = threadIdx.x & 63, l31 = lane & 31, lh = lane >> 5;
+    const int ni = q >> 3, mi = (q >> 2) & 1, a = q & 3;
+    const int m = 32 * mi + l31, n = chunk * SKN_BN + 32 * ni + 8 * a + 4 * lh;
+    if (m >= p.M || n >= p.N) return;
+    const skn_f32x4* src = (const skn_f32x4*)p.sk_work + (long)chunk * (16 * 64) + q * 64 + lane;
+    skn_f32x4 acc = skn_f32x4{0.f, 0.f, 0.f, 0.f};
+    for (int r = 0; r < ranges; ++r) acc += src[(long)r * nchunks * (16 * 64)];
+    skn_epilogue(p, m, n, acc);
+}
+
+extern "C" size_t utx_gemm_skinny_workspace_bytes_impl(const GemmParams* p, int ncu) {
+    if (!p || !skn_shape_ok(p->M, p->N, p->K, p->K2)) return 0;
+    return skn_workspace_bytes(p->N, p->K, ncu);
+}
+
+extern "C" int utx_gemm_skinny_takes(const GemmParams* p, int ncu) {
+    const int tile = g_utx_opt.gemm_tile;
+    if (tile != 0 && tile != 64) return 0;
+    if (!skn_shape_ok(p->M, p->N, p->K, p->K2)) return 0;
+    if (p->mx8 || p->conv_Wo > 0 || p->qk_cols > 0 || p->q_out) return 0;
+    if (tile != 64 && (long)p->N * p->K < SKN_MIN_NK) return 0;
+    if (!p->sk_work || p->sk_work_bytes < skn_workspace_bytes(p->N, p->K, ncu)) return 0;
+    return 1;
+}
+
+extern "C" int utx_launch_gemm_skinny(GemmParams p, int ncu, hipStream_t stream) {
+    const SknPlan s = skn_plan(p.N, p.K, ncu);
+    hipLaunchKernelGGL(gemm_skinny_kernel, dim3(s.nchunks * s.ranges), dim3(256), 0, stream, p, s.nchunks, s.ranges, s.tiles_per_range);
+    hipLaunchKernelGGL(gemm_skinny_fixup_kernel, dim3(s.nchunks * 4), dim3(256), 0, stream, p, s.nchunks, s.ranges);
+    return hipGetLastError() == hipSuccess ? 0 : -4;
+}
diff --git a/unitex_amd/csrc/gemm_skinny_plan.h b/unitex_amd/csrc/gemm_skinny_plan.h
--- /dev/null
+++ b/unitex_amd/csrc/gemm_skinny_plan.h
@@ -0,0 +1,38 @@
+#pragma once
+#include <stddef.h>
+
+#define SKN_BN 64
+#define SKN_BM 64
+#define SKN_BK 64
+#define SKN_MIN_TILES 4
+#define SKN_SLAB_BYTES ((size_t)SKN_BM * SKN_BN * 4)
+#define SKN_MIN_NK (192L * 1024)
+
+struct SknPlan {
+    int nchunks;
+    int ranges;
+    int tiles_per_range;
+};
+
+static inline bool skn_shape_ok(int M, int N, int K, int K2) {
+    return M >= 1 && M <= SKN_BM && N >= 8 && (N % 8) == 0 && K >= SKN_BK && (K % SKN_BK) == 0 && K2 >= 0 && (K2 % SKN_BK) == 0;
+}
+
+static inline SknPlan skn_plan(int N, int K, int ncu) {
+    SknPlan s;
+    s.nchunks = (N + SKN_BN - 1) / SKN_BN;
+    const int nk1 = K / SKN_BK;
+    if (ncu < 1) ncu = 1;
+    int want = (ncu + s.nchunks - 1) / s.nchunks;
+    int most = nk1 / SKN_MIN_TILES;
+    if (most < 1) most = 1;
+    if (want > most) want = most;
+    s.tiles_per_range = (nk1 + want - 1) / want;
+    s.ranges = (nk1 + s.tiles_per_range - 1) / s.tiles_per_range;
+    return s;
+}
+
+static inline size_t skn_workspace_bytes(int N, int K, int ncu) {
+    const SknPlan s = skn_plan(N, K, ncu);
+    return (size_t)s.ranges * (size_t)s.nchunks * SKN_SLAB_BYTES;
+}
diff --git a/unitex_amd/csrc/kernels.h b/unitex_amd/csrc/kernels.h
--- a/unitex_amd/csrc/kernels.h
+++ b/unitex_amd/csrc/kernels.h
@@ -92,6 +92,9 @@
 void utx_gemm_w4_split_plan(const GemmParams* p, int tiles, int grid, int has_work, int* T, int* S);
 int utx_launch_gemm_w4(GemmParams p, hipStream_t stream);
 int utx_launch_gemv_bf16(const GemvParams* p, hipStream_t stream);
+size_t utx_gemm_skinny_workspace_bytes_impl(const GemmParams* p, int ncu);
+int utx_gemm_skinny_takes(const GemmParams* p, int ncu);
+int utx_launch_gemm_skinny(GemmParams p, int ncu, hipStream_t stream);
 int utx_launch_quant_mx8(const void* x, long ldx, void* q, long ldq, void* s, long lds, int M, int K, hipStream_t stream);
 int utx_launch_quant_mx8_packed(const void* x, long ldx, void* q, long ldq, void* s, long row_blocks, int M, int K, hipStream_t stream);
 int utx_launch_qkv_post(const QkvPostParams* p, hipStream_t stream);
diff --git a/unitex_amd/csrc/plan.cpp b/unitex_amd/csrc/plan.cpp
--- a/unitex_amd/csrc/plan.cpp
+++ b/unitex_amd/csrc/plan.cpp
@@ -126,6 +126,16 @@
     int n = 0;
     for (Entry& e : p->entries)
         if (e.kind == K_GEMM && !e.side) { e.gemm.sk_work = sk_work; e.gemm.sk_work_bytes = sk_work_bytes; ++n; }
+    return n;
+}
+
+int utx_plan_assign_sk_txt(utx_plan* p, void* work, size_t work_bytes) {
+    if (!p || !work || !work_bytes) return 0;
+    bool any_side = false;
+    for (const Entry& e : p->entries) if (e.side) any_side = true;
+    int n = 0;
+    for (Entry& e : p->entries)
+        if (e.kind == K_GEMM && e.gemm.M <= 64 && (e.side || !any_side)) { e.gemm.sk_work = work; e.gemm.sk_work_bytes = work_bytes; ++n; }
     return n;
 }
 
diff --git a/unitex_amd/flux/ops.py b/unitex_amd/flux/ops.py
--- a/unitex_amd/flux/ops.py
+++ b/unitex_amd/flux/ops.py
@@ -135,7 +135,7 @@
     return _SK_WS[key]
 
 
-GEMM_KERNELS = ("128x128", "w4")
+GEMM_KERNELS = ("128x128", "w4", None, None, None, "skinny")
 
 
 def gemm_plan(M, N, K=3072, K2=0, n_split=None, gelu_from=None, lora_seg_n=None, lora_n_limit=None, sk=True, n_cus=256):
diff --git a/unitex_amd/flux/transformer.py b/unitex_amd/flux/transformer.py
--- a/unitex_amd/flux/transformer.py
+++ b/unitex_amd/flux/transformer.py
@@ -658,13 +658,28 @@
                 elif e[0] == "par":
                     yield from main_gemms(e[1][0])
         descs = list(main_gemms(plan))
-        if not any(((d.M + 255) // 256) * (d.N // 256) > ncu for d in descs):
+        if any(((d.M + 255) // 256) * (d.N // 256) > ncu for d in descs):
+            if "sk" not in ws:
+                ws["sk"] = ops.streamk_workspace(self.device, shared=False)
+            sk = ws["sk"]
+            for d in descs:
+                d.sk_work, d.sk_work_bytes = ptr(sk), sk.numel()
+
+        def side_gemms(entries):
+            for e in entries:
+                if e[0] == "par":
+                    for s in e[1][1]:
+                        if s[0] is self.lib.utx_gemm_bf16:
+                            yield s[1]
+        if self.fp8_weights:
             return
-        if "sk" not in ws:
-            ws["sk"] = ops.streamk_workspace(self.device, shared=False)
-        sk = ws["sk"]
-        for d in descs:
-            d.sk_work, d.sk_work_bytes = ptr(sk), sk.numel()
+        txt = [d for d in (side_gemms(plan) if any(e[0] == "par" for e in plan) else descs) if d.M <= 64]
+        need = max([int(self.lib.utx_gemm_skinny_workspace_bytes(C.byref(d), int(ncu))) for d in txt] + [0])
+        if need > 0:
+            if "sk_txt" not in ws or ws["sk_txt"].numel() < need:
+                ws["sk_txt"] = torch.empty(need, dtype=torch.uint8, device=self.device)
+            for d in txt:
+                d.sk_work, d.sk_work_bytes = ptr(ws["sk_txt"]), ws["sk_txt"].numel()
 
     TEXT_KEEP = 64
 
@@ -1012,6 +1027,8 @@
         sk, aw = ws.get("sk"), ws.get("attn_ws")
         w.sk_work, w.sk_work_bytes = ptr(sk), 0 if sk is None else sk.numel()
         w.attn_work, w.attn_work_bytes = ptr(aw), 0 if aw is None else aw.numel()
+        skt = ws.get("sk_txt")
+        w.sk_txt_work, w.sk_txt_work_bytes = ptr(skt), 0 if skt is None else skt.numel()
         if self.fp8_weights:
             w.aq, w.as_rm, w.asp, w.asp_row_blocks = ptr(ws["aq"]), ptr(ws["as"]), ptr(ws["asp"]), ws["asp"].stride(0) // 512
             if "aq2" in ws:
```

After: 0.5777, median of 6. About the same (+0.4%).
